# ronghanghu/speaker_follower

Measured on AMD Instinct MI355X. Metric: agent-steps/sec (follower rollout, batch 100), higher is better.
Workload: dtype f32; 1 GPU; follower rollout: batch 100 per GPU, 36 views x 2048-d features from a 10567-viewpoint HBM table, <=80-token instructions, 20 decode steps, argmax (student-forcing) feedback, every step executed for every row (no early exit), encoder included; global_batch=100, parallelism=dp1

## Files before the change

### include/sf_hip.h

```cpp
#ifndef SF_HIP_H_
#define SF_HIP_H_

#include <stddef.h>
#include <stdint.h>

#ifdef __cplusplus
extern "C" {
#endif

#define SF_ABI_VERSION 10

enum {
    SF_OK = 0,
    SF_ERR_ARG = 1,
    SF_ERR_UNSUPPORTED = 2,
    SF_ERR_LAUNCH = 3,
    SF_ERR_WORKSPACE = 4
};

typedef void* sf_stream;

typedef struct sf_dropout {
    float p;
    uint32_t seed;
// ... 397 lines not shown
                    float* logp, sf_stream stream);
int sf_scatter_rows(const float* src, int ld_src, const int32_t* idx, int n, int width, float* dst,
                    int ld_dst, sf_stream stream);

typedef struct sf_spk_beam {
    int32_t B, beam_size, k, T, Tp, eos;
    float* score;
    int64_t* words;
    int32_t* parent;
    int32_t* inst;
    int32_t* live_total;
    int32_t *hist_word, *hist_parent;
    float *hist_score, *hist_attn;
    int64_t ld_hist;
    int32_t* done_rec;
    float* done_score;
} sf_spk_beam;
int sf_speaker_beam_select(const sf_spk_beam* s, const int32_t* top_w, const float* top_lp, const float* alpha,
                           sf_stream stream);

#define SF_ROW_MOVES_MAX 4
typedef struct sf_row_move {
    const float* src;
    float* dst;
    const int32_t* idx;
    int32_t ld_src, ld_dst, width;
    int32_t scatter;
} sf_row_move;
int sf_move_rows(const sf_row_move* moves, int n_moves, int n, sf_stream stream);

int sf_fill_f32(float* p, size_t n, float v, sf_stream stream);
int sf_add_f32(float* dst, const float* src, size_t n, sf_stream stream);
#define SF_FILL_MAX_REGIONS 8
typedef struct sf_fill_region {
    void* ptr;
    uint64_t count;
    uint64_t value;
    int32_t width;
} sf_fill_region;
int sf_fill_regions(const sf_fill_region* regions, int n, sf_stream stream);
int sf_dropout_copy(const float* src, int lds, int B, int N, float* dst, int ldd,
                    const sf_dropout* drop, uint32_t drop_stream, int col0, sf_stream stream);
int sf_transpose(const float* src, int R, int Ccols, float* dst, sf_stream stream);
int sf_embedding_fwd(const float* table, int E, const int64_t* idx, int B, float* out,
                     sf_stream stream);

int sf_adam_step(float* p, const float* g, float* m, float* v, size_t n, double lr, double beta1,
                 double beta2, double eps, double weight_decay, int step, sf_stream stream);
int sf_adam_step_dev(float* p, const float* g, float* m, float* v, size_t n, double lr, double beta1, double beta2,
                     double eps, double weight_decay, int32_t* step_dev, float* coef, const uint32_t* skip_if_nonzero,
                     sf_stream stream);

void sf_debug_trace(unsigned long long* buf);
void sf_debug_force_write_through(int on);
void sf_debug_persist_timeout(long long ticks);
int sf_debug_cotenant(int blocks, int threads, int lds_bytes, long long ticks, float* sink, sf_stream stream);
void sf_gate_product_strict(int on);
int sf_gate_product_is_strict(void);
size_t sf_pack_bf16_bytes(int rows, int K);
int sf_pack_bf16(const float* w, int ld, int rows, int K, void* out, sf_stream stream);
int sf_lstm_weights_bf16(const float* w_ih, const float* w_hh, const void* packed_ih, const void* packed_hh);
void sf_gate_product_bf16_weights(int on);
int sf_gate_product_bf16_weights_is_on(void);
int sf_gate_product_bf16_supported(int M, int K1, int K2, int N);
int sf_feature_table_f16(const void* table, int on);
int sf_feature_table_is_f16(const void* table);
typedef struct sf_projected {
    const float *pv, *pa, *lv, *la;
    const float* loc_table;
    const float *key_v, *key_a;
    int32_t H, ld, V, IMG, LOC, reserved;
} sf_projected;
int sf_projected_ld(int H);
int sf_projected_build(const sf_decoder_fold* fold, const float* table, long long n_rows, const float* loc_table, int V, int IMG,
                       int LOC, int H, float* pv, float* pa, float* lv, float* la, void* ws, size_t ws_bytes,
                       sf_stream stream);
int sf_projected_register(const void* table, const sf_projected* p);
int sf_projected_registered(const void* table, sf_projected* out);
void sf_projected_use(int on);
int sf_projected_is_used(void);
long long sf_projected_steps(void);
int sf_projected_supported(int B, int H, int L, int A, int V, int IMG, int LOC);
void sf_debug_projected_chunk_rows(int rows);
void sf_debug_projected_partials_late(int on);
int sf_projected_text_groups_plan(int B, int L, int with_partials, int slots, int product_blocks, int* grid);
void sf_debug_projected_text_groups(int groups);
int sf_debug_projected_attention(const sf_pano* X, int B, int H, const float* pv, const float* lv, int ld, const float* h1,
                                 int ldh1, float* alpha, float* out, int ldo, int late, void* ws, size_t ws_bytes,
                                 sf_stream stream);
void sf_debug_gate_product_f32(int on);
void sf_debug_many_row_product(int on);
void sf_debug_grouped_weight_gradients(int on);
void sf_debug_slab_consumers(int on);
void sf_debug_precise_attention(int on);
void sf_debug_tn_split_min_rows(int rows);
size_t sf_workspace_fault_offset(size_t ws_bytes);
typedef struct sf_nav_table {
    const int32_t* a_num;
    const int32_t* next_row;
    const int32_t* cand_view;
    const float* cand_sincos;
    const int32_t* feat_row;
    int32_t A, V;
} sf_nav_table;
typedef struct sf_nav_io {
    sf_nav_table nav;
    const int32_t *row, *view;
    const int32_t* goal_hop;
    int32_t ld_hop;
    const int32_t* hop_base;
    int32_t *row_next, *vp_next, *view_next, *a_num_next;
    int32_t* cand_view_next;
    float* sincos_next;
    int64_t* target_next;
} sf_nav_io;
int sf_nav_step(const sf_nav_table* nav, int B, const int32_t* row, const int32_t* view,
                const int64_t* a_t, const uint8_t* ended, const int32_t* goal_hop, int ld_hop,
                const int32_t* hop_base, int32_t* row_next, int32_t* vp_next, int32_t* view_next,
                int32_t* a_num_next, int32_t* cand_view_next, float* sincos_next,
                int64_t* target_next, sf_stream stream);

typedef struct sf_fol_beam {
    int32_t B, beam_size, k, episode_len, T, reserved;
    sf_nav_table nav;
    float* score;
    int32_t *row, *view;
    int32_t* act;
    int32_t* parent;
    int32_t* inst;
    int32_t* live_total;
    int32_t *hist_parent, *hist_action, *hist_rank, *hist_sid, *hist_psid;
    float *hist_score, *hist_attn;
    int64_t ld_hist;
    int32_t* done_rec;
    float* done_score;
} sf_fol_beam;
int sf_follower_beam_select(const sf_fol_beam* s, const int32_t* top_a, const float* top_lp, const float* alpha,
                            sf_stream stream);

enum {
    SF_SEARCH_OVF_NODES = 1, SF_SEARCH_OVF_SLOTS = 2, SF_SEARCH_OVF_VISITS = 4, SF_SEARCH_OVF_POOL = 8,
    SF_SEARCH_OVF_KEY = 16
};
typedef struct sf_state_search {
    int32_t B, successor_size, completion_size, episode_len, key_fields, n_keys;
    int32_t node_cap, slot_cap, visit_cap, cap, pool_rows, reserved;
    sf_nav_table nav;
    const int32_t* base_row;
    int32_t* status;
    int32_t* inst;
    int32_t* frontier;
    int32_t *node_parent, *node_sid, *node_key, *node_action, *node_count, *node_pool, *node_start, *node_born;
    float* node_score;
    int32_t *open_slot, *open_key, *open_node;
    float* open_pick;
    int32_t *held_slot, *held_key, *held_node;
    float* held_pick;
    int32_t* comp_node;
    int32_t* comp_order;
    int32_t* visits;
} sf_state_search;
int sf_state_factored_select(const sf_state_search* s, const float* logp, int ld_logp, int32_t* dev_in,
                             sf_stream stream);

#define SF_EVAL_MAX_NODES 512
typedef struct sf_eval_graphs {
// ... 82 lines not shown
```

### speaker_follower_amd/csrc/sf_api.hip

```cpp
#include "sf_kernels.h"
#include "sf_gemm_small.h"
#include "sf_glue.h"

using namespace sf;

#include <atomic>
#include <climits>
#include <map>
#include <mutex>
#include <string>
#include <vector>

namespace sf {
thread_local hipError_t g_last_hip_error = hipSuccess;

namespace {
struct ProfRec { const char* name; hipEvent_t e0, e1; };
struct Prof {
    std::atomic<bool> active{false};
    std::vector<ProfRec> recs;
    std::vector<hipEvent_t> pool;
    size_t used = 0;
};
Prof g_prof;
std::mutex g_prof_mutex;
}
bool prof_active() { return g_prof.active.load(std::memory_order_acquire); }
void prof_events(const char* name, hipEvent_t* e0, hipEvent_t* e1) {
    std::lock_guard<std::mutex> lock(g_prof_mutex);
    Prof& p = g_prof;
    *e0 = *e1 = nullptr;
    if (!p.active.load(std::memory_order_relaxed)) return;
    while (p.pool.size() < p.used + 2) {
        hipEvent_t e = nullptr;
        if (hipEventCreate(&e) != hipSuccess) { e = nullptr; }
        p.pool.push_back(e);
    }
    if (!p.pool[p.used] || !p.pool[p.used + 1]) return;
    *e0 = p.pool[p.used++];
    *e1 = p.pool[p.used++];
    p.recs.push_back(ProfRec{name, *e0, *e1});
}
}

namespace {

constexpr size_t WORKSPACE_BYTES = 64u << 20;
constexpr size_t WGRAD_WORKSPACE_BYTES = 256u << 20;

struct Arena {
    float* base;
    size_t cap, off;
    unsigned* tk = nullptr;
    float* take(size_t n) {
        n = (n + 63) & ~(size_t)63;
        if (off + n > cap) return nullptr;
        float* p = base + off;
        off += n;
        return p;
    }
    float* rest() const { return base + off; }
    size_t rest_n() const { return cap - off; }
    unsigned* tickets() const { return tk; }
};
constexpr size_t SYNC_WORDS = 2048;
constexpr size_t PERSIST_TICKET = 1100;
constexpr size_t TEXT_TICKET = 1200;

inline Arena arena(void* ws, size_t bytes) {
    const size_t n = ws ? bytes / 4 : 0;
    const size_t usable = n > SYNC_WORDS ? n - SYNC_WORDS : 0;
    return Arena{(float*)ws, usable, 0, usable ? reinterpret_cast<unsigned*>((float*)ws + usable) : nullptr};
}
inline hipStream_t S(sf_stream s) { return (hipStream_t)s; }

constexpr int F16_TABLES = 16;
const void* g_f16_tables[F16_TABLES];
int g_f16_ntables = 0;
std::mutex g_f16_mutex;
int table_is_f16(const void* table) {
    if (!table) return 0;
    std::lock_guard<std::mutex> lock(g_f16_mutex);
    for (int i = 0; i < g_f16_ntables; ++i)
        if (g_f16_tables[i] == table) return 1;
    return 0;
}

constexpr int PROJ_TABLES = 16;
struct ProjEntry { const void* table; sf_projected p; };
ProjEntry g_proj[PROJ_TABLES];
int g_proj_n = 0;
std::mutex g_proj_mutex;
std::atomic<int> g_proj_use{1};
std::atomic<long long> g_proj_steps{0};
static int g_proj_partials_late = 0;
bool projected_lookup(const void* table, sf_projected* out) {
    if (!table || !g_proj_use.load(std::memory_order_relaxed)) return false;
    std::lock_guard<std::mutex> lock(g_proj_mutex);
    for (int i = 0; i < g_proj_n; ++i)
        if (g_proj[i].table == table) {
            *out = g_proj[i].p;
            return true;
        }
    return false;
}
inline int projected_ld(int H) { return (H + 1 + 3) & ~3; }

inline PanoSrc pano(const sf_pano* p) {
    return PanoSrc{p->dense, p->table, p->loc_table, p->vp, p->view, p->V, p->IMG, p->LOC,
                   p->dense ? 0 : table_is_f16(p->table)};
}
inline CandSrc cands(const sf_cands* c) {
    return CandSrc{c->dense, c->table, c->vp, c->cand_view, c->cand_sincos, c->a_num,
                   c->A, c->V, c->IMG, c->LOC, c->dense ? 0 : table_is_f16(c->table)};
}

inline FGlue make_glue(const CandSrc& src, int B, float* logit, const sf_follower_glue* g) {
    FGlue f{};
    f.src = src; f.B = B; f.logit = logit; f.is_valid = g->is_valid; f.target = g->target;
    f.feedback = g->feedback; f.ended = g->ended; f.a_t = g->a_t; f.target_used = g->target_used;
    f.score = g->score; f.u_next = g->u_next; f.ld_u = g->ld_u_next;
    f.u_drop = make_dropout(g->u_drop, g->u_drop_stream, 2);
    f.ce_term = g->ce_term; f.live = g->live; f.sample_seed = g->sample_seed;
    f.sample_stream = g->sample_stream; f.row0 = g->row0;
    f.sample_site = g->sample_site_dev ? g->sample_site_dev : site_zero();
    if (g->nav) {
        const sf_nav_io& n = *g->nav;
        f.nav = NavIO{n.nav, n.row, n.view, n.goal_hop, n.ld_hop, n.hop_base, n.row_next, n.vp_next, n.view_next,
                      n.a_num_next, n.cand_view_next, n.sincos_next, n.target_next, true};
    }
    return f;
}
inline bool glue_ok(const sf_cands* U, const sf_follower_glue* g) {
    return g->target && g->ended && g->a_t && g->target_used && g->score && g->ce_term && g->live &&
           g->feedback >= 0 && g->feedback <= 2 && (g->is_valid || U->a_num) &&
           (!g->u_next || g->ld_u_next % 4 == 0) &&
           (!g->nav || (g->nav->nav.A == U->A && g->nav->nav.a_num && g->nav->nav.next_row && g->nav->nav.cand_view &&
                        g->nav->nav.cand_sincos && g->nav->nav.feat_row && g->nav->row && g->nav->view &&
                        g->nav->row_next && g->nav->vp_next && g->nav->view_next && g->nav->a_num_next &&
                        g->nav->cand_view_next && g->nav->sincos_next &&
                        (!g->nav->target_next || (g->nav->goal_hop && g->nav->hop_base && g->nav->ld_hop > 0))));
}

#define TRY(expr)                     \
    do {                              \
        int _st = (expr);             \
        if (_st != SF_OK) return _st; \
    } while (0)
#define NEED(ptr) \
    if (!(ptr)) return SF_ERR_WORKSPACE

int colsum_pair(const float* Y, int ldy, int M, int N, float* a, float* b, Arena ar, hipStream_t st) {
    float* first = a ? a : b;
    if (!first) return SF_OK;
    return colsum(Y, ldy, M, N, first, 1, st, (a && b) ? b : nullptr, ar.rest(), ar.rest_n());
}

int linear_plain(const float* x, int ldx, const float* w, int ldw, const float* b, int M, int N,
                 int K, Epi epi, float* y, int ldy, Arena ar, hipStream_t st) {
    Seg sg{x, ldx, w, ldw, K};
    LinearOut o{};
    o.y = y;
    o.ldy = ldy;
    o.bias = b;
    o.epi = epi;
    return linear_nt(&sg, 1, M, N, o, ar.rest(), ar.rest_n(), st);
}

int data_grad(const float* dy, int lddy, const float* w, const float* w_t, int M, int N, int K,
              float* dx, int lddx, int accumulate, Arena ar, hipStream_t st) {
    if (w_t && N % 4 == 0) {
        Seg sg{dy, lddy, w_t, N, N};
        LinearOut o{};
        o.y = dx; o.ldy = lddx; o.epi = EPI_NONE; o.accumulate = accumulate;
        return linear_nt(&sg, 1, M, K, o, ar.rest(), ar.rest_n(), st);
    }
    return gemm_nn_ws(dy, lddy, w, K, M, K, N, dx, lddx, accumulate, ar.rest(), ar.rest_n(), st);
}

std::atomic<int> g_bf16w_on{0};
struct Bf16Pair { const float* w_ih; const float* w_hh; const void* p_ih; const void* p_hh; };
constexpr int BF16_PAIRS = 16;
Bf16Pair g_bf16_pairs[BF16_PAIRS];
int g_bf16_npairs = 0;
std::mutex g_bf16_mutex;

bool bf16_packed(const float* w_ih, const float* w_hh, const void* (&packed)[2]) {
    if (!g_bf16w_on.load(std::memory_order_relaxed) || sf::g_nt_force_f32) return false;
    std::lock_guard<std::mutex> lock(g_bf16_mutex);
    for (int i = 0; i < g_bf16_npairs; ++i)
        if (g_bf16_pairs[i].w_ih == w_ih && g_bf16_pairs[i].w_hh == w_hh) {
            packed[0] = g_bf16_pairs[i].p_ih;
            packed[1] = g_bf16_pairs[i].p_hh;
            return true;
        }
    return false;
}

int lstm_fwd_i(const sf_lstm_w* w, int B, int I, int H, const float* x, int ldx, const float* h0,
               const float* c0, float* h1, float* c1, float* gates, float* h1_drop, int ld_h1_drop,
               const Dropout& drop, Arena ar, hipStream_t st) {
    LstmPwFwd p{};
    p.xg = nullptr; p.b_ih = w->b_ih; p.b_hh = w->b_hh;
    p.c0 = c0; p.h0 = h0; p.B = B; p.H = H; p.gates = gates; p.h1 = h1; p.c1 = c1;
    p.h1_drop = h1_drop; p.ld_h1_drop = ld_h1_drop; p.drop = drop; p.lengths = nullptr;
    if (I + H <= 1024 && H % 16 == 0) {
        LstmStepArgs f{};
        f.h0 = h0; f.w_hh = w->w_hh; f.x = x; f.ldx = ldx; f.w_ih = w->w_ih; f.I = I; f.xg = nullptr;
        f.b_ih = w->b_ih; f.b_hh = w->b_hh; f.B = B; f.H = H; f.pw = p;
        return lstm_step_fused(f, st);
    }
    Seg segs[2] = {{x, ldx, w->w_ih, I, I}, {h0, H, w->w_hh, H, H}};
    LinearOut o{};
    float* slabs = nullptr;
    int ks = 1;
    const void* packed[2];
    const bool bf16w = bf16_packed(w->w_ih, w->w_hh, packed);
    TRY(linear_nt(segs, 2, B, 4 * H, o, ar.rest(), ar.rest_n(), st, &slabs, &ks, bf16w ? packed : nullptr));
    p.slabs = slabs; p.ks = ks;
    return lstm_pointwise_fwd(p, st);
}

static int g_slab_consumers = 1;

int lstm_bwd_i(const sf_lstm_w* w, const sf_lstm_g* g, int B, int I, int H, const float* x, int ldx,
               const float* h0, const float* c0, const float* c1, const float* gates,
               const float* dh1, const float* dh1_b, const float* dc1, float* dx, int lddx,
               float* dh0, float* dc0, Arena ar, hipStream_t st, float* dgates_out = nullptr,
               int dx_col0 = 0,
               const Dropout* dh1b_drop = nullptr,
               SmallPlan* dh0_plan = nullptr, bool* dh0_deferred = nullptr,
               const float** dx_slabs = nullptr, int* dx_ks = nullptr) {
    float* dgates = dgates_out ? dgates_out : ar.take((size_t)B * 4 * H);
    NEED(dgates);
    LstmPwBwd p{};
    p.gates = gates; p.c0 = c0; p.c1 = c1; p.dh1 = dh1; p.dh1_b = dh1_b; p.dc1 = dc1;
    p.B = B; p.H = H; p.dgates = dgates; p.dc0 = dc0; p.lengths = nullptr; p.dh0_pass = nullptr;
    if (dh1b_drop) p.dh1b_drop = *dh1b_drop;
    TRY(lstm_pointwise_bwd(p, st));
    if (dx && dx_col0 == 0) {
        TRY(data_grad(dgates, 4 * H, w->w_ih, w->w_ih_t, B, 4 * H, I, dx, lddx, 0, ar, st));
    } else if (dx) {
        const int I2 = I - dx_col0;
        if (dx_ks) *dx_ks = 0;
        if (w->w_ih_t) {
            Seg sg{dgates, 4 * H, w->w_ih_t + (size_t)dx_col0 * 4 * H, 4 * H, 4 * H};
            LinearOut o{};
            o.y = dx + dx_col0; o.ldy = lddx; o.epi = EPI_NONE;
            float* slabs = (dx_slabs && dx_ks && g_slab_consumers) ? ar.take((size_t)16 * B * I2) : nullptr;
            int ks = 0;
            float* raw = nullptr;
            if (slabs && linear_nt(&sg, 1, B, I2, o, slabs, (size_t)16 * B * I2, st, &raw, &ks) == SF_OK && raw == slabs && ks >= 1) {
                *dx_slabs = slabs;
                *dx_ks = ks;
            } else {
                TRY(linear_nt(&sg, 1, B, I2, o, ar.rest(), ar.rest_n(), st));
            }
        } else {
            TRY(gemm_nn_ws(dgates, 4 * H, w->w_ih + dx_col0, I, B, I2, 4 * H, dx + dx_col0, lddx, 0,
                           ar.rest(), ar.rest_n(), st));
        }
    }
    if (dh0_deferred) *dh0_deferred = false;
    if (dh0 && dh0_plan && dh0_deferred && w->w_hh_t) {
        Seg sg{dgates, 4 * H, w->w_hh_t, 4 * H, 4 * H};
        LinearOut o{};
        o.y = dh0; o.ldy = H; o.epi = EPI_NONE;
        *dh0_deferred = linear_small_plan(&sg, 1, B, H, o, dh0_plan);
    }
    if (dh0 && !(dh0_deferred && *dh0_deferred))
        TRY(data_grad(dgates, 4 * H, w->w_hh, w->w_hh_t, B, 4 * H, H, dh0, H, 0, ar, st));
    if (g) {
        if (g->w_ih) TRY(gemm_tn(dgates, 4 * H, x, ldx, B, 4 * H, I, g->w_ih, I, 1, st, ar.rest(), ar.rest_n()));
        if (g->w_hh) TRY(gemm_tn(dgates, 4 * H, h0, H, B, 4 * H, H, g->w_hh, H, 1, st, ar.rest(), ar.rest_n()));
        TRY(colsum_pair(dgates, 4 * H, B, 4 * H, g->b_ih, g->b_hh, ar, st));
    }
    return SF_OK;
}

int visual_fwd_i(const sf_visual_w* w, const PanoSrc& X, int B, int H, int D, const float* h,
                 float* out, int ldo, float* alpha, float* t_v, float* q, const Dropout& drop,
                 int col0, Arena ar, hipStream_t st, bool precise = false, const sf_visual_fold64* fold64 = nullptr) {
    const int F = X.IMG + X.LOC;
    if (precise && fold64 && fold64->m_v && fold64->c_v && visual_attn_f64_supported(X, B) && !(H & 3)) {
        double* q64 = reinterpret_cast<double*>(ar.take((size_t)B * F * 2));
        float* part = ar.take(visual_attn_split_floats(B, F));
        if (q64 && part && ar.tickets()) {
            TRY(linear_f64_w64(h, H, fold64->m_v, H, fold64->c_v, B, F, H, q64, F, q, F, st));
            return visual_attn(0, X, B, q, F, alpha, out, ldo, drop, col0, st, part, ar.tickets(), q64);
        }
    }
    if (precise && w->w_v_t && visual_attn_f64_supported(X, B) && !(H & 3) && !(D & 3)) {
        double* t64 = reinterpret_cast<double*>(ar.take((size_t)B * D * 2));
        double* q64 = reinterpret_cast<double*>(ar.take((size_t)B * F * 2));
        float* part = ar.take(visual_attn_split_floats(B, F));
        if (t64 && q64 && part && ar.tickets()) {
            TRY(linear_f64(h, nullptr, H, w->w_h, H, w->b_h, B, D, H, t64, D, t_v, D, st));
            TRY(linear_f64(nullptr, t64, D, w->w_v_t, D, nullptr, B, F, D, q64, F, q, F, st));
            return visual_attn(0, X, B, q, F, alpha, out, ldo, drop, col0, st, part, ar.tickets(), q64);
        }
// ... 228 lines not shown
        if (g_proj_n == PROJ_TABLES) return SF_ERR_UNSUPPORTED;
        at = g_proj_n++;
    }
    g_proj[at] = ProjEntry{table, *p};
    return SF_OK;
}
int sf_projected_registered(const void* table, sf_projected* out) {
    std::lock_guard<std::mutex> lock(g_proj_mutex);
    for (int i = 0; i < g_proj_n; ++i)
        if (table && g_proj[i].table == table) {
            if (out) *out = g_proj[i].p;
            return 1;
        }
    return 0;
}
void sf_projected_use(int on) { g_proj_use.store(on ? 1 : 0, std::memory_order_relaxed); }
int sf_projected_is_used(void) { return g_proj_use.load(std::memory_order_relaxed); }
long long sf_projected_steps(void) { return g_proj_steps.load(std::memory_order_relaxed); }
void sf_debug_projected_partials_late(int on) { g_proj_partials_late = on; }
void sf_debug_projected_text_groups(int groups) { sf::g_proj_text_groups = groups == 2 || groups == 4 ? groups : 0; }
int sf_projected_text_groups_plan(int B, int L, int with_partials, int slots, int product_blocks, int* grid) {
    if (B < 1 || L < 1 || slots < 0 || product_blocks < 0) return 0;
    return sf::proj_text_groups_plan(B, L, with_partials != 0, product_blocks, slots, 0, grid);
}
int sf_debug_projected_attention(const sf_pano* X, int B, int H, const float* pv, const float* lv, int ld, const float* h1,
                                 int ldh1, float* alpha, float* out, int ldo, int late, void* ws, size_t ws_bytes,
                                 sf_stream stream) {
    SF_ENTER();
    SF_CHECK_ARG(X && pv && lv && h1 && alpha && out && B > 0 && H > 0);
    const PanoSrc x = pano(X);
    Arena ar = arena(ws, ws_bytes);
    float* part = ar.take(visual_attn_split_floats(B, x.IMG + x.LOC));
    if (!part || !ar.tickets()) return SF_ERR_WORKSPACE;
    return proj_attention_alone(x, B, ProjTables{pv, nullptr, lv, nullptr, ld, H}, h1, ldh1, alpha, out, ldo, late, part,
                                ar.tickets(), S(stream));
}
constexpr long long PROJ_CHUNK_ROWS = 16384;
static long long g_proj_chunk_rows = PROJ_CHUNK_ROWS;
void sf_debug_projected_chunk_rows(int rows) { g_proj_chunk_rows = rows > 0 ? rows : PROJ_CHUNK_ROWS; }
int sf_projected_supported(int B, int H, int L, int A, int V, int IMG, int LOC) {
    if (H <= 0 || IMG <= 0 || LOC <= 0 || V <= 0) return 0;
    static const float dummy[4] = {0.f, 0.f, 0.f, 0.f};
    static const int idummy[1] = {0};
    CandSrc us{};
    us.table = dummy; us.a_num = idummy; us.A = A; us.V = V; us.IMG = IMG; us.LOC = LOC;
    PanoSrc xn{};
    xn.table = dummy; xn.V = V; xn.IMG = IMG; xn.LOC = LOC;
    const ProjTables pt{dummy, dummy, dummy, dummy, projected_ld(H), H};
    return proj_chain_supported(us, &xn, B, H, L, pt) ? 1 : 0;
}
int sf_projected_build(const sf_decoder_fold* fold, const float* table, long long n_rows, const float* loc_table, int V, int IMG,
                       int LOC, int H, float* pv, float* pa, float* lv, float* la, void* ws, size_t ws_bytes,
                       sf_stream stream) {
    SF_ENTER();
    SF_CHECK_ARG(fold && fold->m_v && fold->c_v && fold->m_a && fold->c_a && table && loc_table && pv && pa && lv && la &&
                 n_rows > 0 && V > 0 && IMG > 0 && IMG % 4 == 0 && LOC > 0 && LOC % 16 == 0 && H > 0 && H % 4 == 0);
    if (table_is_f16(table)) return SF_ERR_UNSUPPORTED;
    const int F = IMG + LOC, Fa = F + 4, ld = projected_ld(H), Ks = LOC + 4, g = LOC / 4;
    Arena ar = arena(ws, ws_bytes);
    hipStream_t st = S(stream);
    sf::proj_text_slots_warm();
    float* wt_v = ar.take((size_t)ld * F);
    float* wt_a = ar.take((size_t)ld * Fa);
    float* sel = ar.take((size_t)5 * Ks);
    NEED(wt_v && wt_a && sel);
    TRY(fill(wt_v + (size_t)H * F, (size_t)(ld - H) * F, 0.f, st));
    TRY(fill(wt_a + (size_t)H * Fa, (size_t)(ld - H) * Fa, 0.f, st));
    TRY(transpose(fold->m_v, F, H, wt_v, st));
    TRY(transpose(fold->m_a, Fa, H, wt_a, st));
    TRY(add2(fold->c_v, F, nullptr, 0, 1, F, wt_v + (size_t)H * F, F, st));
    TRY(add2(fold->c_a, Fa, nullptr, 0, 1, Fa, wt_a + (size_t)H * Fa, Fa, st));
    TRY(fill(sel, (size_t)5 * Ks, 0.f, st));
    for (int q = 0; q < 4; ++q) TRY(fill(sel + (size_t)q * Ks + (size_t)q * g, (size_t)g, 1.f, st));
    TRY(fill(sel + (size_t)4 * Ks + LOC, 1, 1.f, st));
    for (long long r0 = 0; r0 < n_rows; r0 += g_proj_chunk_rows) {
        const int m = (int)std::min<long long>(g_proj_chunk_rows, n_rows - r0);
        const float* x = table + (size_t)r0 * IMG;
        TRY(linear_plain(x, IMG, wt_v, F, nullptr, m, ld, IMG, EPI_NONE, pv + (size_t)r0 * ld, ld, ar, st));
        TRY(linear_plain(x, IMG, wt_a, Fa, nullptr, m, ld, IMG, EPI_NONE, pa + (size_t)r0 * ld, ld, ar, st));
    }
    TRY(linear_plain(loc_table, LOC, wt_v + IMG, F, nullptr, V * V, ld, LOC, EPI_NONE, lv, ld, ar, st));
    return linear_plain(sel, Ks, wt_a + IMG, Fa, nullptr, 5, ld, Ks, EPI_NONE, la, ld, ar, st);
}
void sf_gate_product_bf16_weights(int on) { g_bf16w_on.store(on ? 1 : 0, std::memory_order_relaxed); }
int sf_gate_product_bf16_weights_is_on(void) { return g_bf16w_on.load(std::memory_order_relaxed); }
int sf_gate_product_bf16_supported(int M, int K1, int K2, int N) {
    if (K2 < 0) return 0;
    const int K[2] = {K1, K2};
    return sf::bf16w_supported(M, N, K, K2 ? 2 : 1) ? 1 : 0;
}
void sf_debug_precise_attention(int on) { sf::g_precise_attention = on; }
void sf_debug_tn_split_min_rows(int rows) { sf::g_tn_split_min_rows = rows < 0 ? 4096 : rows; }
size_t sf_workspace_fault_offset(size_t ws_bytes) {
    const size_t n = ws_bytes / 4;
    if (n <= SYNC_WORDS) return 0;
    return (n - SYNC_WORDS + PERSIST_TICKET + persistent_fault_word()) * 4;
}
const char* sf_last_error_string(void) { return hipGetErrorString(g_last_hip_error); }
const char* sf_status_string(int s) {
    switch (s) {
        case SF_OK: return "ok";
        case SF_ERR_ARG: return "invalid argument";
        case SF_ERR_UNSUPPORTED: return "unsupported shape";
        case SF_ERR_LAUNCH: return "kernel launch failed";
        case SF_ERR_WORKSPACE: return "workspace too small";
        default: return "unknown status";
    }
}

int sf_linear_fwd(const float* x, int ldx, const float* w, const float* b, int M, int N, int K,
                  int act, float* y, int ldy, void* ws, size_t ws_bytes, sf_stream stream) {
    SF_ENTER();
    SF_CHECK_ARG(x && w && y && M > 0 && N > 0 && K > 0 && (act == 0 || act == 1));
    return linear_plain(x, ldx, w, K, b, M, N, K, act ? EPI_TANH : EPI_NONE, y, ldy,
                        arena(ws, ws_bytes), S(stream));
}

int sf_linear_slabs_fwd(const float* x, int ldx, const float* w, int K1, const float* h, int ldh,
                        const float* u, int K2, int M, int N, int* ksplit, void* ws, size_t ws_bytes,
                        sf_stream stream) {
    SF_ENTER();
    SF_CHECK_ARG(x && w && ksplit && ws && M > 0 && N > 0 && K1 > 0 && (!h || (u && K2 > 0)));
    Arena ar = arena(ws, ws_bytes);
    Seg segs[2] = {{x, ldx, w, K1, K1}, {h, ldh, u, K2, K2}};
    LinearOut o{};
    float* slabs = nullptr;
    const void* packed[2];
    const bool bf16w = bf16_packed(w, h ? u : nullptr, packed);
    return linear_nt(segs, h ? 2 : 1, M, N, o, ar.rest(), ar.rest_n(), S(stream), &slabs, ksplit, bf16w ? packed : nullptr);
}

int sf_linear_bwd(const float* x, int ldx, const float* w, const float* y, int ldy, const float* dy,
                  int lddy, int M, int N, int K, int act, float* dx, int lddx, int accumulate_dx,
                  float* dw, float* db, void* ws, size_t ws_bytes, sf_stream stream) {
    SF_ENTER();
    SF_CHECK_ARG(x && w && dy && M > 0 && N > 0 && K > 0 && (N % 4 == 0) && (K % 4 == 0));
    Arena ar = arena(ws, ws_bytes);
    hipStream_t st = S(stream);
    const float* dpre = dy;
    int ldp = lddy;
    if (act == 1) {
        SF_CHECK_ARG(y);
        float* t = ar.take((size_t)M * N);
        NEED(t);
        TRY(tanh_bwd(y, ldy, dy, lddy, M, N, t, N, st));
        dpre = t;
        ldp = N;
    }
    if (dx) TRY(gemm_nn_ws(dpre, ldp, w, K, M, K, N, dx, lddx, accumulate_dx, ar.rest(), ar.rest_n(), st));
    if (dw) TRY(gemm_tn(dpre, ldp, x, ldx, M, N, K, dw, K, 1, st, ar.rest(), ar.rest_n()));
    if (db) TRY(colsum(dpre, ldp, M, N, db, 1, st, nullptr, ar.rest(), ar.rest_n()));
    return SF_OK;
}

int sf_lstm_cell_fwd(const sf_lstm_w* w, int B, int I, int H, const float* x, int ldx,
                     const float* h0, const float* c0, float* h1, float* c1, float* gates,
                     float* h1_drop, int ld_h1_drop, const sf_dropout* drop, uint32_t drop_stream,
                     void* ws, size_t ws_bytes, sf_stream stream) {
    SF_ENTER();
    SF_CHECK_ARG(w && x && h0 && c0 && h1 && c1 && B > 0 && I > 0 && H > 0 && H % 4 == 0);
    return lstm_fwd_i(w, B, I, H, x, ldx, h0, c0, h1, c1, gates, h1_drop, ld_h1_drop,
                      make_dropout(drop, drop_stream), arena(ws, ws_bytes), S(stream));
}

int sf_lstm_cell_bwd(const sf_lstm_w* w, const sf_lstm_g* g, int B, int I, int H, const float* x,
                     int ldx, const float* h0, const float* c0, const float* c1, const float* gates,
// ... 68 lines not shown
    SF_ENTER();
    SF_CHECK_ARG(w && ctx && alpha && cat2 && t_text && h_tilde && dh_tilde && dh && B > 0);
    return softdot_bwd_i(w, g, B, L, H, ctx, alpha, cat2, t_text, h_tilde, dh_tilde, dh, lddh, dctx,
                         arena(ws, ws_bytes), S(stream));
}

int sf_text_attention_fwd(const float* ctx, const uint8_t* mask, int B, int L, int H, const float* t, int ldt,
                          float* alpha, float* wc, int ldwc, sf_stream stream) {
    SF_ENTER();
    SF_CHECK_ARG(ctx && t && alpha && wc && B > 0 && L > 0 && H > 0);
    return text_attn_fwd(ctx, mask, B, L, H, t, ldt, alpha, wc, ldwc, S(stream));
}

int sf_text_attention_bwd(const float* ctx, int B, int L, int H, const float* dwc, int lddwc, const float* t, int ldt,
                          const float* alpha, float* dt, int lddt, float* dctx, sf_stream stream) {
    SF_ENTER();
    SF_CHECK_ARG(ctx && dwc && t && alpha && dt && B > 0 && L > 0 && H > 0);
    return text_attn_bwd(ctx, B, L, H, dwc, lddwc, t, ldt, alpha, dt, lddt, dctx, S(stream));
}

int sf_eltwise_prod_scoring_fwd(const sf_scoring_w* w, const sf_cands* U, int B, int H, int D,
                                const float* h, float* logit, float* t_a, float* wt, float* r,
                                void* ws, size_t ws_bytes, sf_stream stream) {
    SF_ENTER();
    SF_CHECK_ARG(w && U && h && logit && t_a && wt && r && B > 0);
    return scoring_fwd_i(w, cands(U), B, H, D, h, logit, t_a, wt, r, arena(ws, ws_bytes), S(stream));
}

int sf_eltwise_prod_scoring_bwd(const sf_scoring_w* w, const sf_scoring_g* g, const sf_cands* U,
                                int B, int H, int D, const float* h, const float* t_a,
                                const float* wt, const float* dlogit, float* dh, void* ws,
                                size_t ws_bytes, sf_stream stream) {
    SF_ENTER();
    SF_CHECK_ARG(w && U && h && t_a && wt && dlogit && B > 0);
    return scoring_bwd_i(w, g, cands(U), B, H, D, h, t_a, wt, dlogit, dh, arena(ws, ws_bytes),
                         S(stream));
}

static int decoder_head_a(const sf_decoder_w* w, const sf_pano* X, int B, int H, int D,
                          const float* h0, const sf_decoder_tape* tp, const sf_dropout* drop,
                          uint32_t step_id, Arena ar, sf_stream stream) {
    SF_CHECK_ARG(w && X && h0 && tp && B > 0);
    const PanoSrc xs = pano(X);
    const int F = xs.IMG + xs.LOC;
    return visual_fwd_i(&w->visual, xs, B, H, D, h0, tp->xin + F, 2 * F, tp->alpha_v, tp->t_v, tp->q,
                        make_dropout(drop, 2 * step_id, 2), F, ar, S(stream));
}

int sf_attn_decoder_head_fwd(const sf_decoder_w* w, const sf_pano* X, int B, int H, int D,
                             const float* h0, const sf_decoder_tape* tp, const sf_dropout* drop,
                             uint32_t step_id, void* ws, size_t ws_bytes, sf_stream stream) {
    SF_ENTER();
    return decoder_head_a(w, X, B, H, D, h0, tp, drop, step_id, arena(ws, ws_bytes), stream);
}

static int plan_linear(const float* x, int ldx, const float* wgt, int ldw, const float* b, int M,
                       int N, int K, Epi epi, float* y, int ldy, SmallPlan* p) {
    Seg sg{x, ldx, wgt, ldw, K};
    LinearOut o{};
    o.y = y; o.ldy = ldy; o.bias = b; o.epi = epi;
    return linear_small_plan(&sg, 1, M, N, o, p) ? SF_OK : SF_ERR_UNSUPPORTED;
}

struct TextFold {
    const float* ctx_q;
    const float* ctx_o;
};

struct TailStep {
    const sf_decoder_w* w;
    CandSrc us;
    int B, H, D, L, F;
    const sf_decoder_tape *tp, *tn;
    const sf_follower_glue* glue;
    Dropout d_h, dn_in;
    PanoSrc xn;
    bool has_xn;
    bool paired, query_only, last_step;
    const float* ctx;
    const uint8_t* ctx_mask;
    const int32_t* ctx_row;
    Arena ar;
    hipStream_t st;
};

static inline int issued(int rc) { return rc == SF_ERR_UNSUPPORTED ? SF_ERR_LAUNCH : rc; }

static SmallPlan empty_plan(SmallPlan p) {
    p.gx = p.gy = 0;
    return p;
}

static int vis_next_beside(const TailStep& s, float* part, unsigned* counter, const SmallPlan& b, int phase = 0) {
    return pair_vis_small(s.xn, s.B, s.tn->q, s.F, s.tn->alpha_v, s.tn->xin + s.F, 2 * s.F, s.dn_in, s.F, part, counter, b,
                          s.st, phase);
}
static int vis_next_alone(const TailStep& s, float* part, const Arena& ar) {
    return visual_attn(0, s.xn, s.B, s.tn->q, s.F, s.tn->alpha_v, s.tn->xin + s.F, 2 * s.F, s.dn_in, s.F, s.st, part,
                       part ? ar.tickets() : nullptr);
}

static int score_tail(const TailStep& s, const Arena& ar, bool t_a_done = false) {
    const sf_decoder_tape* tp = s.tp;
    return scoring_fwd_i(&s.w->action, s.us, s.B, s.H, s.D, tp->h_tilde, tp->logit, tp->t_a, tp->wt, tp->r, ar, s.st, s.glue,
                         t_a_done);
}

struct FoldScratch {
    float *tpart, *ybuf, *zbuf, *part;
    unsigned* tcount;
    int ldp;
    bool ok;
};
static FoldScratch fold_scratch(const TailStep& s, Arena& af) {
    FoldScratch f{};
    f.tpart = af.take(text_fold_part_floats(s.B, s.H));
    f.ldp = s.H + 16;
    f.ybuf = af.take((size_t)s.B * f.ldp);
    f.zbuf = af.take((size_t)s.B * f.ldp);
    f.tcount = af.tickets() ? af.tickets() + TEXT_TICKET : nullptr;
    f.part = (s.paired && s.B <= 1024) ? af.take(visual_attn_split_floats(s.B, s.F)) : nullptr;
    f.ok = f.tpart && f.ybuf && f.zbuf && (f.part || !s.paired) && f.tcount && s.B <= VIS_SPLIT_MAX_B;
    return f;
}

static int fold_score(const TailStep& s, float* merge_part) {
    const sf_scoring_w& a = s.w->action;
    const sf_decoder_tape* tp = s.tp;
    if (merge_part)
        return pair_score_merge(s.us, s.B, s.D, tp->r, tp->wt, a.b_a, a.b_out, make_glue(s.us, s.B, tp->logit, s.glue), s.xn,
                                s.tn->alpha_v, s.tn->xin + s.F, 2 * s.F, s.dn_in, s.F, merge_part, s.st);
    if (s.glue)
        return score_glue_fwd(s.us, s.B, s.D, tp->r, tp->wt, a.b_a, a.b_out, make_glue(s.us, s.B, tp->logit, s.glue), s.st);
    return score_fwd(s.us, s.B, s.D, tp->r, tp->wt, a.b_a, a.b_out, tp->logit, s.st);
}

static bool projected_for(const sf_decoder_w* w, const CandSrc& us, const PanoSrc* xn, int B, int H, int L, ProjTables* pt) {
    sf_projected reg;
    if (us.dense || us.half || !projected_lookup(us.table, &reg)) return false;
    if (reg.key_v != w->visual.w_h || reg.key_a != w->action.w_h || reg.V != us.V || reg.IMG != us.IMG || reg.LOC != us.LOC ||
        (xn && xn->loc_table != reg.loc_table))
        return false;
    *pt = ProjTables{reg.pv, reg.pa, reg.lv, reg.la, reg.ld, reg.H};
    return proj_chain_supported(us, xn, B, H, L, *pt);
}

static int tail_proj(const TailStep& s, const TextFold& tf) {
    const sf_decoder_tape *tp = s.tp, *tn = s.tn;
    const int B = s.B, H = s.H, F = s.F;
    ProjTables pt;
    if (!s.glue || s.query_only || !(s.paired || s.last_step) ||
        !projected_for(s.w, s.us, s.paired ? &s.xn : nullptr, B, H, s.L, &pt))
        return SF_ERR_UNSUPPORTED;
    Arena af = s.ar;
    const FoldScratch f = fold_scratch(s, af);
    SmallPlan py;
    const bool ok = f.ok &&
        plan_linear(tp->cat2 + H, 2 * H, s.w->text.w_out + H, 2 * H, nullptr, B, H, H, EPI_NONE, f.ybuf, f.ldp, &py) == SF_OK &&
        pair_proj_textfold_accepts(py.inst()) && (!s.paired || af.tickets());
    if (!ok) return SF_ERR_UNSUPPORTED;
    const bool late = s.paired && (g_proj_partials_late || !proj_partials_supported(s.xn.IMG, s.xn.LOC));
    TRY(pair_proj_textfold(tf.ctx_q, tf.ctx_o, s.ctx_mask, B, s.L, H, tp->cat2 + H, 2 * H, f.tpart, f.tcount, f.zbuf, f.ldp,
                           tp->alpha, py, s.us, s.paired && !late ? &s.xn : nullptr, pt, tp->h1, H, f.part, s.st));
    g_proj_steps.fetch_add(1, std::memory_order_relaxed);
    return issued(pair_proj_score(s.us, B, H, s.L, pt, f.zbuf, f.ldp, f.ybuf, f.ldp, make_glue(s.us, B, tp->logit, s.glue),
                                  s.paired ? &s.xn : nullptr, late ? 0 : 2, tp->h1, H, s.paired ? tn->alpha_v : nullptr,
                                  s.paired ? tn->xin + F : nullptr, 2 * F, s.dn_in, F, f.part, af.tickets(), s.st));
}

static int tail_fold4(const TailStep& s, const TextFold& tf) {
    const sf_visual_w* vw = &s.w->visual;
    const sf_scoring_w* aw = &s.w->action;
    const sf_decoder_tape *tp = s.tp, *tn = s.tn;
    const int B = s.B, H = s.H, D = s.D, F = s.F;
    Arena af = s.ar;
    const FoldScratch f = fold_scratch(s, af);
    SmallPlan py, pv, pta, pq, pr;
    bool ok = f.ok &&
        plan_linear(tp->cat2 + H, 2 * H, s.w->text.w_out + H, 2 * H, nullptr, B, H, H, EPI_NONE, f.ybuf, f.ldp, &py) == SF_OK &&
        plan_linear(tp->wt, D, aw->w_a_t, D, nullptr, B, F, D, EPI_NONE, tp->r, F, &pr) == SF_OK;
    if (ok && !s.last_step) {
        ok = plan_linear(tp->h1, H, vw->w_h, H, vw->b_h, B, D, H, EPI_NONE, tn->t_v, D, &pv) == SF_OK &&
             plan_linear(tn->t_v, D, vw->w_v_t, D, nullptr, B, F, D, EPI_NONE, tn->q, F, &pq) == SF_OK;
    } else if (ok) {
        pv = empty_plan(py);
        pq = empty_plan(pr);
    }
    if (ok) {
        Seg sg{f.ybuf, f.ldp, aw->w_h, H, H};
        LinearOut o{};
        o.y = tp->wt; o.ldy = D; o.bias = aw->b_h; o.mul = aw->w_out; o.y_pre = tp->t_a;
        o.ldy_pre = D; o.epi = EPI_MUL;
        ok = linear_small_plan(&sg, 1, B, D, o, &pta) && pair_apro_small_accepts(pta.inst(), pq.inst()) &&
             pair_vis_small_accepts(pr.inst(), 1);
        pta.args.apro_part = f.zbuf;
        pta.args.apro_stride = f.ldp;
    }
    if (!ok) return SF_ERR_UNSUPPORTED;
    TRY(pair_textfold_small_small(tf.ctx_q, tf.ctx_o, s.ctx_mask, B, s.L, H, tp->cat2 + H, 2 * H, f.tpart, f.tcount, f.zbuf,
                                  f.ldp, tp->alpha, py, pv, s.st));
    TRY(issued(pair_apro_small(pta, pq, s.st)));
    const bool merge_late = s.paired && s.glue;
    if (merge_late) TRY(issued(vis_next_beside(s, f.part, nullptr, pr, 1)));
    else if (s.paired) TRY(issued(vis_next_beside(s, f.part, af.tickets(), pr, 0)));
    else TRY(issued(launch_small_plan(pr, s.st)));
    return issued(fold_score(s, merge_late ? f.part : nullptr));
}

static int text_and_query(const TailStep& s) {
    const sf_softdot_w* tw = &s.w->text;
    const sf_visual_w* vw = &s.w->visual;
    const sf_decoder_tape *tp = s.tp, *tn = s.tn;
    const int B = s.B, H = s.H, D = s.D, L = s.L, F = s.F;
    SmallPlan pa, pb;
    const bool ok1 =
        plan_linear(tp->cat2 + H, 2 * H, tw->w_in, H, nullptr, B, H, H, EPI_NONE, tp->t_text, H, &pa) == SF_OK &&
        plan_linear(tp->h1, H, vw->w_h, H, vw->b_h, B, D, H, EPI_NONE, tn->t_v, D, &pb) == SF_OK;
    if (!ok1 || pair_small_small(pa, pb, s.st) != SF_OK) {
        TRY(linear_plain(tp->cat2 + H, 2 * H, tw->w_in, H, nullptr, B, H, H, EPI_NONE, tp->t_text, H, s.ar, s.st));
        TRY(linear_plain(tp->h1, H, vw->w_h, H, vw->b_h, B, D, H, EPI_NONE, tn->t_v, D, s.ar, s.st));
    }
    const bool ok2 = plan_linear(tn->t_v, D, vw->w_v_t, D, nullptr, B, F, D, EPI_NONE, tn->q, F, &pa) == SF_OK;
    if (!ok2 || pair_small_text(pa, s.ctx, s.ctx_mask, B, L, H, tp->t_text, H, tp->alpha, tp->cat2,
                                2 * H, s.ctx_row, s.st) != SF_OK) {
        TRY(text_attn_fwd(s.ctx, s.ctx_mask, B, L, H, tp->t_text, H, tp->alpha, tp->cat2, 2 * H, s.st, s.ctx_row));
        TRY(linear_plain(tn->t_v, D, vw->w_v_t, D, nullptr, B, F, D, EPI_NONE, tn->q, F, s.ar, s.st));
    }
    return SF_OK;
}

static int tail_paired(const TailStep& s) {
    const sf_softdot_w* tw = &s.w->text;
    const sf_scoring_w* aw = &s.w->action;
    const sf_decoder_tape* tp = s.tp;
    const int B = s.B, H = s.H, D = s.D, F = s.F;
    Arena ar = s.ar;
    float* part = B <= 1024 ? ar.take(visual_attn_split_floats(B, F)) : nullptr;
    SmallPlan ph, pc;
    const bool ok3 = part && plan_linear(tp->cat2, 2 * H, tw->w_out, 2 * H, nullptr, B, H, 2 * H,
                                         EPI_TANH, tp->h_tilde, H, &ph) == SF_OK;
    bool ok4 = false;
    if (ok3) {
        Seg sg{tp->h_tilde, H, aw->w_h, H, H};
        LinearOut o{};
        o.y = tp->wt; o.ldy = D; o.bias = aw->b_h; o.mul = aw->w_out; o.y_pre = tp->t_a;
        o.ldy_pre = D; o.epi = EPI_MUL;
        ok4 = linear_small_plan(&sg, 1, B, D, o, &pc) && pair_vis_small_accepts(pc.inst(), 2);
    }
    TRY(text_and_query(s));
    if (ok4 && vis_next_beside(s, part, nullptr, ph, 1) == SF_OK) {
        TRY(vis_next_beside(s, part, nullptr, pc, 2));
        return score_tail(s, ar, true);
    }
    if (!ok3 || vis_next_beside(s, part, ar.tickets(), ph) != SF_OK) {
        TRY(linear_plain(tp->cat2, 2 * H, tw->w_out, 2 * H, nullptr, B, H, 2 * H, EPI_TANH, tp->h_tilde, H, ar, s.st));
        TRY(vis_next_alone(s, part, ar));
    }
    return score_tail(s, ar);
}

static int tail_query_only(const TailStep& s) {
    const sf_decoder_tape* tp = s.tp;
    TRY(text_and_query(s));
    TRY(linear_plain(tp->cat2, 2 * s.H, s.w->text.w_out, 2 * s.H, nullptr, s.B, s.H, 2 * s.H, EPI_TANH, tp->h_tilde, s.H,
                     s.ar, s.st));
    return score_tail(s, s.ar);
}

static int tail_plain(const TailStep& s) {
    const sf_decoder_tape *tp = s.tp, *tn = s.tn;
    TRY(softdot_fwd_i(&s.w->text, s.B, s.L, s.H, nullptr, 0, s.ctx, s.ctx_mask, tp->h_tilde, tp->alpha, tp->cat2,
                      tp->t_text, s.ar, s.st, s.ctx_row));
    if (s.has_xn)
        TRY(visual_fwd_i(&s.w->visual, s.xn, s.B, s.H, s.D, tp->h1, tn->xin + s.F, 2 * s.F, tn->alpha_v, tn->t_v, tn->q,
                         s.dn_in, s.F, s.ar, s.st));
    return score_tail(s, s.ar);
}

static int tail_dispatch(const TailStep& s, const TextFold* tf) {
    const bool foldable = (s.paired || s.query_only || s.last_step) && tf && !s.ctx_row && !s.d_h.on() && s.w->text.w_out;
    int rc = SF_ERR_UNSUPPORTED;
    if (foldable) rc = tail_proj(s, *tf);
    if (rc == SF_ERR_UNSUPPORTED && foldable && s.w->action.w_a_t) rc = tail_fold4(s, *tf);
    if (rc != SF_ERR_UNSUPPORTED) return rc;
    if (s.paired) return tail_paired(s);
    if (s.query_only) return tail_query_only(s);
    return tail_plain(s);
}

static int decoder_tail_i(const sf_decoder_w* w, const sf_cands* U, int B, int H, int D, int L,
                          const float* u_prev, const float* h0, const float* c0, const float* ctx,
                          const uint8_t* ctx_mask, const int32_t* ctx_row, const sf_decoder_tape* tp,
                          const sf_follower_glue* glue, const sf_dropout* drop, uint32_t step_id,
                          const sf_pano* X_next, const sf_decoder_tape* tn, void* ws, size_t ws_bytes,
                          sf_stream stream, const TextFold* tf = nullptr) {
    SF_CHECK_ARG(w && U && h0 && c0 && ctx && tp && B > 0 && L > 0 && (!glue || glue_ok(U, glue)) &&
                 (!X_next || tn));
    TailStep s{};
    s.w = w; s.us = cands(U); s.B = B; s.H = H; s.D = D; s.L = L; s.F = s.us.IMG + s.us.LOC;
    s.tp = tp; s.tn = tn; s.glue = glue;
    s.ctx = ctx; s.ctx_mask = ctx_mask; s.ctx_row = ctx_row;
    s.ar = arena(ws, ws_bytes);
    s.st = S(stream);
    s.d_h = make_dropout(drop, 2 * step_id + 1, 2);
    s.dn_in = make_dropout(drop, 2 * (step_id + 1), 2);
    s.has_xn = X_next != nullptr;
    if (X_next) s.xn = pano(X_next);
    s.paired = X_next && w->visual.w_v_t;
    s.query_only = !X_next && tn && w->visual.w_v_t;
    s.last_step = !X_next && !tn;
    const Dropout d_in = make_dropout(drop, 2 * step_id, 2);
    if (u_prev) TRY(dropout_copy(u_prev, s.F, B, s.F, tp->xin, 2 * s.F, d_in, 0, s.st));
    TRY(lstm_fwd_i(&w->lstm, B, 2 * s.F, H, tp->xin, 2 * s.F, h0, c0, tp->h1, tp->c1, tp->gates,
                   tp->cat2 + H, 2 * H, s.d_h, s.ar, s.st));
    return tail_dispatch(s, tf);
}

static int decoder_tail_split_i(const sf_decoder_w* w, const sf_cands* U, int B, int H, int D, int L,
                                const float* h0, const float* c0, const float* ctx, const uint8_t* ctx_mask,
                                const sf_decoder_tape* tp, const sf_follower_glue* glue, const sf_dropout* drop,
                                uint32_t step_id, unsigned* flag_h1, unsigned flag_value, void* ws,
                                size_t ws_bytes, unsigned* tickets, hipStream_t st) {
    SF_CHECK_ARG(w && U && h0 && c0 && ctx && tp && glue && glue_ok(U, glue));
    const size_t n = ws_bytes / 4;
    Arena ar{(float*)ws, n, 0, tickets};
    const CandSrc us = cands(U);
    const int F = us.IMG + us.LOC;
    const Dropout d_h = make_dropout(drop, 2 * step_id + 1, 2);
    TRY(lstm_fwd_i(&w->lstm, B, 2 * F, H, tp->xin, 2 * F, h0, c0, tp->h1, tp->c1, tp->gates, tp->cat2 + H, 2 * H,
                   d_h, ar, st));
    if (flag_h1) TRY(flag_set(flag_h1, flag_value, st));
    TRY(softdot_fwd_i(&w->text, B, L, H, nullptr, 0, ctx, ctx_mask, tp->h_tilde, tp->alpha, tp->cat2, tp->t_text,
                      ar, st, nullptr));
    return scoring_fwd_i(&w->action, us, B, H, D, tp->h_tilde, tp->logit, tp->t_a, tp->wt, tp->r, ar, st, glue);
}

int sf_attn_decoder_attend_fwd(const sf_pano* X, int B, const sf_decoder_tape* tp, const sf_dropout* drop,
                               uint32_t step_id, void* ws, size_t ws_bytes, sf_stream stream) {
    SF_ENTER();
    SF_CHECK_ARG(X && tp && tp->q && tp->xin && tp->alpha_v && B > 0);
    Arena ar = arena(ws, ws_bytes);
    const PanoSrc xs = pano(X);
    const int F = xs.IMG + xs.LOC;
    float* part = B <= 1024 ? ar.take(visual_attn_split_floats(B, F)) : nullptr;
    return visual_attn(0, xs, B, tp->q, F, tp->alpha_v, tp->xin + F, 2 * F, make_dropout(drop, 2 * step_id, 2), F,
                       S(stream), part, part ? ar.tickets() : nullptr);
}

int sf_attn_decoder_tail_fwd(const sf_decoder_w* w, const sf_cands* U, int B, int H, int D, int L,
                             const float* u_prev, const float* h0, const float* c0,
                             const float* ctx, const uint8_t* ctx_mask, const int32_t* ctx_row,
                             const sf_decoder_tape* tp, const sf_follower_glue* glue,
                             const sf_dropout* drop, uint32_t step_id, const sf_pano* X_next,
                             const sf_decoder_tape* tn, void* ws, size_t ws_bytes,
                             sf_stream stream) {
    SF_ENTER();
    return decoder_tail_i(w, U, B, H, D, L, u_prev, h0, c0, ctx, ctx_mask, ctx_row, tp, glue, drop,
                          step_id, X_next, tn, ws, ws_bytes, stream);
}

int sf_attn_decoder_fwd(const sf_decoder_w* w, const sf_pano* X, const sf_cands* U, int B, int H,
                        int D, int L, const float* u_prev, const float* h0, const float* c0,
                        const float* ctx, const uint8_t* ctx_mask, const int32_t* ctx_row,
                        const sf_decoder_tape* tp, const sf_follower_glue* glue,
                        const sf_dropout* drop, uint32_t step_id,
                        void* ws, size_t ws_bytes, sf_stream stream) {
    SF_ENTER();
    SF_CHECK_ARG(w && X && U && h0 && c0 && ctx && tp && B > 0 && L > 0 && (!glue || glue_ok(U, glue)));
    TRY(decoder_head_a(w, X, B, H, D, h0, tp, drop, step_id, arena(ws, ws_bytes), stream));
    return decoder_tail_i(w, U, B, H, D, L, u_prev, h0, c0, ctx, ctx_mask, ctx_row, tp, glue, drop, step_id, nullptr,
                          nullptr, ws, ws_bytes, stream);
}

int sf_decoder_fold_build(const sf_decoder_w* w, int H, int D, int F, float* m_v, float* c_v,
                          float* m_a, float* c_a, void* ws, size_t ws_bytes, sf_stream stream) {
    SF_ENTER();
    SF_CHECK_ARG(w && m_v && c_v && m_a && c_a && w->visual.w_v_t && w->visual.w_h_t &&
                 w->action.w_a_t && w->action.w_h_t && F % 4 == 0 && D % 4 == 0 && H % 4 == 0);
    Arena ar = arena(ws, ws_bytes);
    hipStream_t st = S(stream);
    float* wa_s = ar.take((size_t)F * D);
    float* wo_ba = ar.take(D);
    float* wo_bh = ar.take(D);
    NEED(wa_s && wo_ba && wo_bh);
    TRY(linear_plain(w->visual.w_v_t, D, w->visual.w_h_t, D, nullptr, F, H, D, EPI_NONE, m_v, H, ar, st));
    TRY(linear_plain(w->visual.b_h, D, w->visual.w_v_t, D, nullptr, 1, F, D, EPI_NONE, c_v, F, ar, st));
    TRY(scale_cols(w->action.w_a_t, D, w->action.w_out, F, D, wa_s, D, st));
    TRY(scale_cols(w->action.b_a, D, w->action.w_out, 1, D, wo_ba, D, st));
    TRY(scale_cols(w->action.b_h, D, w->action.w_out, 1, D, wo_bh, D, st));
    TRY(fill(m_a + (size_t)F * H, (size_t)4 * H, 0.f, st));
    TRY(fill(c_a + F, 4, 0.f, st));
    TRY(linear_plain(wa_s, D, w->action.w_h_t, D, nullptr, F, H, D, EPI_NONE, m_a, H, ar, st));
    TRY(linear_plain(wo_ba, D, w->action.w_h_t, D, nullptr, 1, H, D, EPI_NONE, m_a + (size_t)F * H, H, ar, st));
    TRY(linear_plain(wo_bh, D, w->action.w_a_t, D, nullptr, 1, F, D, EPI_NONE, c_a, F + 4, ar, st));
    return linear_plain(wo_bh, D, w->action.b_a, D, w->action.b_out, 1, 1, D, EPI_NONE, c_a + F, 4, ar, st);
}

// ... 197 lines not shown
        side = side_st;
        ev_join = ev_back;
        return SF_OK;
    }
    int join() {
        hipStream_t from = side;
        side = nullptr;
        return order_behind(main, from, ev_join);
    }
    ~SideFork() { if (side) (void)join(); }
};
}
}

int sf_follower_episode_fwd(const sf_decoder_w* w, const sf_follower_episode* e, void* ws,
                            size_t ws_bytes, sf_stream stream) {
    SF_ENTER();
    SF_CHECK_ARG(w && e && e->S > 0 && e->B > 0 && e->h_init && e->c_init && e->ctx && e->tape.xin &&
                 e->tape.h1 && e->tape.c1 && e->glue.target && e->glue.ended);
    const sf_dropout* drop = e->drop.p > 0.f ? &e->drop : nullptr;
    StepView cur = step_view(e, 0);
    TextFold tfold{e->ctx_q, e->ctx_o};
    const TextFold* tf = nullptr;
    if (e->ctx_q && e->ctx_o && !drop && e->S > 1 && w->text.w_in_t && w->text.w_out && w->action.w_a_t) {
        const int M = e->B * e->L, H = e->H;
        const Arena ar = arena(ws, ws_bytes);
        TRY(linear_plain(e->ctx, H, w->text.w_in_t, H, nullptr, M, H, H, EPI_NONE, e->ctx_q, H, ar, S(stream)));
        TRY(linear_plain(e->ctx, H, w->text.w_out, 2 * H, nullptr, M, H, H, EPI_NONE, e->ctx_o, H, ar, S(stream)));
        tf = &tfold;
    }
    {
        Arena ha = arena(ws, ws_bytes);
        const PanoSrc x0 = pano(&cur.X);
        ProjTables pt;
        float* part = nullptr;
        bool head_done = false;
        if (tf && !e->glue.nav && e->B <= VIS_SPLIT_MAX_B && projected_for(w, cands(&cur.U), &x0, e->B, e->H, e->L, &pt) &&
            (part = ha.take(visual_attn_split_floats(e->B, x0.IMG + x0.LOC))) && ha.tickets()) {
            const int F = x0.IMG + x0.LOC;
            const int rc = visual_attn_proj(cands(&cur.U), x0, e->B, e->H, e->L, pt, e->h_init, e->H, cur.tp.alpha_v,
                                            cur.tp.xin + F, 2 * F, make_dropout(drop, 2 * e->step0, 2), F, part, ha.tickets(),
                                            S(stream));
            if (rc == SF_OK) head_done = true;
            else if (rc != SF_ERR_UNSUPPORTED) return rc;
        }
        if (!head_done)
            TRY(decoder_head_a(w, &cur.X, e->B, e->H, e->D, e->h_init, &cur.tp, drop, e->step0, ha, stream));
    }
    const sf_nav_io* nav0 = e->glue.nav;
    if (nav0) SF_CHECK_ARG(w->visual.w_v_t);
    if (!nav0 && e->side_stream && e->side_stream != stream && e->S > 1 && !tf) {
        hipStream_t ms = S(stream), ss = S(e->side_stream);
        std::vector<hipEvent_t>& ev = event_pool(2);
        if (ev.size() < 2) return SF_ERR_LAUNCH;
        const Arena whole = arena(ws, ws_bytes);
        if (!whole.tk) return SF_ERR_WORKSPACE;
        const size_t side_n = std::min<size_t>(whole.cap / 4, (size_t)4 << 20);
        unsigned* flag_h1 = whole.tk + PERSIST_TICKET + 48;
        unsigned* flag_ft = whole.tk + PERSIST_TICKET + 49;
        void* side_ws = (float*)ws + (whole.cap - side_n);
        const size_t main_bytes = (whole.cap - side_n) * sizeof(float);
        TRY(flag_set(flag_h1, 0u, ms));
        TRY(flag_set(flag_ft, 0u, ms));
        SideFork fk{ms};
        TRY(fk.fork(ss, ev[0], ev[1]));
        for (int t = 0; t < e->S; ++t) {
            const bool more = t + 1 < e->S;
            StepView nxt = more ? step_view(e, t + 1) : cur;
            const StepState in = state_in(e, t);
            if (t > 0) TRY(flag_wait(flag_ft, (unsigned)t, ms));
            TRY(decoder_tail_split_i(w, &cur.U, e->B, e->H, e->D, e->L, in.h, in.c, e->ctx, e->ctx_mask, &cur.tp,
                                     &cur.glue, drop, e->step0 + t, more ? flag_h1 : nullptr, (unsigned)(t + 1), ws,
                                     main_bytes, whole.tk, ms));
            if (more) {
                TRY(flag_wait(flag_h1, (unsigned)(t + 1), ss));
                Arena sar{(float*)side_ws, side_n, 0, whole.tk};
                TRY(decoder_head_a(w, &nxt.X, e->B, e->H, e->D, cur.tp.h1, &nxt.tp, drop, e->step0 + t + 1, sar, e->side_stream));
                TRY(flag_set(flag_ft, (unsigned)(t + 1), ss));
            }
            cur = nxt;
        }
        return fk.join();
    }
    for (int t = 0; t < e->S; ++t) {
        const bool more = t + 1 < e->S;
        StepView nxt = more ? step_view(e, t + 1) : cur;
        const sf_nav_io nv = nav0 ? nav_view(nav0, e, t) : sf_nav_io{};
        if (nav0) cur.glue.nav = &nv;
        const StepState in = state_in(e, t);
        TRY(decoder_tail_i(w, &cur.U, e->B, e->H, e->D, e->L, nullptr, in.h, in.c, e->ctx, e->ctx_mask,
                           nullptr, &cur.tp, &cur.glue, drop, e->step0 + t, more && !nav0 ? &nxt.X : nullptr,
                           more ? &nxt.tp : nullptr, ws, ws_bytes, stream, tf));
        if (nav0 && more)
            TRY(sf_attn_decoder_attend_fwd(&nxt.X, e->B, &nxt.tp, drop, e->step0 + t + 1, ws, ws_bytes, stream));
        cur = nxt;
    }
    return SF_OK;
}

int sf_follower_episode_bwd(const sf_decoder_w* w, const sf_follower_episode* e,
                            const sf_decoder_gtape* gtape, const float* gscale, float* dlogit,
                            float* dh_a, float* dc_a, float* dh_b, float* dc_b, float* dctx,
                            int* result_in_b, void* ws, size_t ws_bytes, sf_stream stream) {
    SF_ENTER();
    SF_CHECK_ARG(w && e && gtape && gscale && dlogit && dh_a && dc_a && dh_b && dc_b && result_in_b &&
                 e->S > 0 && e->B > 0);
    const sf_dropout* drop = e->drop.p > 0.f ? &e->drop : nullptr;
    sf_decoder_gtape gt_all = *gtape;
    if (!(gt_all.dcat2 && gt_all.ds && dctx && ctx_grad_supported(e->S, e->L, e->H)))
        gt_all.dcat2 = gt_all.ds = nullptr;
    gtape = &gt_all;
    const float *dh1 = nullptr, *dc1 = nullptr;
    float *dho = dh_a, *dco = dc_a, *dhn = dh_b, *dcn = dc_b;
    hipStream_t main_st = S(stream), side_st = S(e->side_stream);
    const bool two = side_st && side_st != main_st && gtape->dh1d && gtape->dcat2 && gtape->ds &&
                     e->B <= VIS_SPLIT_MAX_B;
    if (two) {
        SF_CHECK_ARG(e->ctx && dctx);
        std::vector<hipEvent_t>& ev = event_pool(e->S + 1);
        if (ev.size() < (size_t)e->S + 1) return SF_ERR_LAUNCH;
        const Arena whole = arena(ws, ws_bytes);
        const size_t usable = whole.cap;
        const size_t head_n = std::min<size_t>(usable / 4, (size_t)4 << 20);
        Arena tail_ar{(float*)ws, usable - head_n, 0, whole.tk};
        Arena head_ar{(float*)ws + (usable - head_n), head_n, 0, whole.tk};
        TRY(order_behind(side_st, main_st, ev[e->S]));
        for (int t = e->S - 1; t >= 0; --t) {
            StepView v = step_view(e, t);
            const sf_decoder_gtape g = gtape_view(gtape, e, t);
            const CeSrc ce{v.tp.logit, v.glue.target_used, gscale + t, -1, (int)e->A};
            TRY(decoder_bwd_head_i(w, nullptr, &v.U, e->B, e->H, e->D, e->L, e->ctx, &v.tp, &g, dlogit,
                                   g.dh1d, dctx, head_ar, side_st, &ce));
            if (hipEventRecord(ev[t], side_st) != hipSuccess) return SF_ERR_LAUNCH;
        }
        for (int t = e->S - 1; t >= 0; --t) {
            StepView v = step_view(e, t);
            const sf_decoder_gtape g = gtape_view(gtape, e, t);
            const StepState in = state_in(e, t);
            if (hipStreamWaitEvent(main_st, ev[t], 0) != hipSuccess) return SF_ERR_LAUNCH;
            TRY(decoder_bwd_tail_i(w, nullptr, &v.X, e->B, e->H, e->D, in.h, in.c, &v.tp, &g, dh1, g.dh1d, dc1,
                                   dho, dco, drop, e->step0 + t, tail_ar, main_st));
            dh1 = dho;
            dc1 = dco;
            std::swap(dho, dhn);
            std::swap(dco, dcn);
        }
    } else {
        for (int t = e->S - 1; t >= 0; --t) {
            StepView v = step_view(e, t);
            const sf_decoder_gtape g = gtape_view(gtape, e, t);
            const StepState in = state_in(e, t);
            const CeSrc ce{v.tp.logit, v.glue.target_used, gscale + t, -1, (int)e->A};
            TRY(decoder_bwd_i(w, nullptr, &v.X, &v.U, e->B, e->H, e->D, e->L, in.h, in.c, e->ctx, &v.tp, &g,
                              dlogit, dh1, dc1, dho, dco, dctx, drop, e->step0 + t, ws, ws_bytes, stream,
                              &ce));
            dh1 = dho;
            dc1 = dco;
            std::swap(dho, dhn);
            std::swap(dco, dcn);
        }
    }
    *result_in_b = (dh1 == dh_b) ? 1 : 0;
    if (gtape->dcat2 && gtape->ds && dctx)
        TRY(ctx_grad_accum(e->tape.alpha, gtape->ds, gtape->dcat2, 2 * e->H, e->tape.t_text, e->S, e->B,
                           e->L, e->H, dctx, S(stream)));
    return SF_OK;
}

int sf_attn_decoder_wgrad(const sf_decoder_w* w, const sf_decoder_g* g, int M, int H, int D, int F,
                          const float* h0_all, const sf_decoder_tape* tp, const sf_decoder_gtape* gt,
                          void* ws, size_t ws_bytes, sf_stream stream) {
    SF_ENTER();
    SF_CHECK_ARG(w && g && h0_all && tp && gt && M > 0);
    hipStream_t st = S(stream);
    Arena ar = arena(ws, ws_bytes);
// ... 980 lines not shown
```

### speaker_follower_amd/csrc/sf_attention.hip

```cpp
#include <atomic>
#include "sf_kernels.h"
#include "sf_rows.h"
#include "sf_glue.h"
#include "sf_gemm_small.h"

namespace sf {

namespace {


struct VisArgs {
    PanoSrc src;
    const float* vec;
    int ldvec;
    float* alpha;
    float* out;
    int ldo;
    Dropout drop;
    int drop_col0;
    const double* vec64;
    int vec_slabs;
    long vec_slab_stride;
    const float* pv;
    const float* lv;
// ... 823 lines not shown
        dlv = a.logit[(size_t)b * A + min(lane, A - 1)];
    }
    const CandRow row = cand_row<H16>(a.src, b, wave);
    float4 p[SC_CPL];
#pragma unroll
    for (int i = 0; i < SC_CPL; ++i) p[i] = f4zero();
    if (wave < A && !row.zero && w != 0.f) {
#pragma unroll
        for (int i = 0; i < SC_CPL; ++i) {
            const int c = lane + 64 * i;
            f4fma(p[i], w, cand_load<H16>(row, c, c < n4, n4));
        }
    }
    if (wave == 0) {
        const float tot = wave_sum(lane < A ? dlv : 0.f);
        if (lane == 0) a.dc[b] = tot;
    }
    float* orow = a.dr + (size_t)b * (n4 << 2);
    block_row_sum<SC_CPL, SC_NW, SC_SLOTS>(p, slots, n4, [&](int c, float4 t) {
        reinterpret_cast<float4*>(orow)[c] = t;
    });
}

template <int MTA, int CPWA, int MTB, int CPWB>
__global__ __launch_bounds__(SMALL_WAVES * 64) void pair_small_small_kernel(SmallArgs a, int gxa,
                                                                           int na, SmallArgs b,
                                                                           int gxb) {
    const int bid = blockIdx.x;
    if (bid < na)
        small_gemm_body<MTA, CPWA>(a, bid % gxa, bid / gxa);
    else
        small_gemm_body<MTB, CPWB>(b, (bid - na) % gxb, (bid - na) / gxb);
}

template <int MT, int CPW, int RPW>
__global__ __launch_bounds__(TXT_NW * 64) void pair_small_text_kernel(SmallArgs a, int gxa, int na,
                                                                      TxtArgs t) {
    const int bid = blockIdx.x;
    if (bid < na) {
        if (threadIdx.x >= SMALL_WAVES * 64) return;
        small_gemm_body<MT, CPW>(a, bid % gxa, bid / gxa);
    } else {
        text_attn_body<RPW, 0>(t, bid - na);
    }
}

template <int MT, int CPW, int PHASE, bool APRO = false, bool H16 = false>
__global__ __launch_bounds__(SMALL_WAVES * 64) void pair_vis_small_kernel(VisArgs v, VisSplit sp,
                                                                         int nv, SmallArgs b,
                                                                         int gxb) {
    const int bid = blockIdx.x;
    if (bid < nv) {
        if (threadIdx.x >= VSP_NW * 64) return;
        if (PHASE == 2)
            visual_split_body<2>(v, sp, 0, bid);
        else
            visual_split_body<PHASE, false, H16>(v, sp, bid % VSP_G, bid / VSP_G);
    } else {
        small_gemm_body<MT, CPW, false, APRO>(b, (bid - nv) % gxb, (bid - nv) / gxb);
    }
}


template <bool H16>
__global__ __launch_bounds__(SC_NW * 64) void pair_score_merge_kernel(ScoreArgs a, FGlue g, int nb, VisArgs v, VisSplit sp) {
    const int bid = blockIdx.x;
    if (bid < nb) {
        score_glue_body<H16>(a, g, bid);
    } else {
        if (threadIdx.x >= VSP_NW * 64) return;
        visual_split_body<2>(v, sp, 0, bid - nb);
    }
}


struct ProjScoreArgs {
    CandSrc src;
    const float* pa;
    const float* la;
    int ldp, H;
    const float* z;
    const float* y;
    int ldz, ldy;
};

__device__ __forceinline__ void proj_score_glue_body(const ProjScoreArgs& a, const FGlue& g, int b) {
    constexpr int NW = SMALL_WAVES, SLOTS = 2;
    __shared__ float s_logit[64];
    __shared__ int s_at;
    const int tid = threadIdx.x, lane = tid & 63, wave = tid >> 6;
    const int A = a.src.A, V = a.src.V, H = a.H, n4h = H >> 2;
    const size_t ldp = (size_t)a.ldp;
    const FGlueIn gin = follower_glue_load(g, b);
    const int vp = a.src.vp[b], an = a.src.a_num[b];
    const int cvl = a.src.cand_view[(size_t)b * A + min(lane, A - 1)];
    const float4 scl = reinterpret_cast<const float4*>(a.src.cand_sincos)[(size_t)b * A + min(lane, A - 1)];
    float4 zv[PRJ_CPL], yv[PRJ_CPL], lav[5][PRJ_CPL], pav[SLOTS][PRJ_CPL];
    float lac[5], pac[SLOTS];
#pragma unroll
    for (int i = 0; i < PRJ_CPL; ++i) {
        const int cc = min(lane + 64 * i, n4h - 1);
        zv[i] = reinterpret_cast<const float4*>(a.z + (size_t)b * a.ldz)[cc];
        yv[i] = reinterpret_cast<const float4*>(a.y + (size_t)b * a.ldy)[cc];
#pragma unroll
        for (int q = 0; q < 5; ++q) lav[q][i] = reinterpret_cast<const float4*>(a.la + q * ldp)[cc];
    }
#pragma unroll
    for (int q = 0; q < 5; ++q) lac[q] = a.la[q * ldp + H];
#pragma unroll
    for (int k = 0; k < SLOTS; ++k) {
        const int view = __shfl(cvl, min(wave + NW * k, A - 1), WAVE);
        const float* pr = a.pa + ((size_t)max(vp, 0) * V + min(max(view, 0), V - 1)) * ldp;
#pragma unroll
        for (int i = 0; i < PRJ_CPL; ++i) pav[k][i] = reinterpret_cast<const float4*>(pr)[min(lane + 64 * i, n4h - 1)];
        pac[k] = pr[H];
    }
    float4 ht[PRJ_CPL];
#pragma unroll
    for (int i = 0; i < PRJ_CPL; ++i) ht[i] = lane + 64 * i < n4h ? apro_form(yv[i], zv[i]) : f4zero();
#pragma unroll
    for (int k = 0; k < SLOTS; ++k) {
        const int ac = wave + NW * k, acc = min(ac, A - 1);
        const float s0 = __shfl(scl.x, acc, WAVE), s1 = __shfl(scl.y, acc, WAVE), s2 = __shfl(scl.z, acc, WAVE),
                    s3 = __shfl(scl.w, acc, WAVE);
        const float hm = (ac < A && ac != 0 && ac < an && vp >= 0) ? 1.f : 0.f;
        float d = 0.f;
#pragma unroll
        for (int i = 0; i < PRJ_CPL; ++i) {
            float4 w = pav[k][i];
            f4fma(w, s0, lav[0][i]);
            f4fma(w, s1, lav[1][i]);
            f4fma(w, s2, lav[2][i]);
            f4fma(w, s3, lav[3][i]);
            float4 t = lav[4][i];
            f4fma(t, hm, w);
            d += dot4(t, ht[i]);
        }
        d = wave_sum(d);
        const float cst = lac[4] + hm * (pac[k] + s0 * lac[0] + s1 * lac[1] + s2 * lac[2] + s3 * lac[3]);
        if (lane == 0 && ac < A) s_logit[ac] = d + cst;
    }
    __syncthreads();
    if (wave == 0) {
        const int at = follower_glue_row(g, b, lane < A ? s_logit[lane] : 0.f, gin);
        if (lane == 0) s_at = at;
        if (g.nav.on && lane < A) nav_advance_slot(g.nav, b, lane, at, gin.was_ended || at == 0);
    }
    __syncthreads();
    if (g.u_next) {
        const int at = min(max(s_at, 0), A - 1);
        const int n4 = (a.src.IMG + a.src.LOC) >> 2;
        CandRow row;
        row.zero = at == 0 || at >= an || vp < 0;
        row.I4 = a.src.IMG >> 2;
        row.g4 = max(a.src.LOC >> 4, 1);
        const int view = __shfl(cvl, at, WAVE);
        row.img = reinterpret_cast<const float4*>(a.src.table) + ((size_t)max(vp, 0) * V + min(max(view, 0), V - 1)) * row.I4;
        row.img16 = nullptr;
        row.s0 = __shfl(scl.x, at, WAVE); row.s1 = __shfl(scl.y, at, WAVE);
        row.s2 = __shfl(scl.z, at, WAVE); row.s3 = __shfl(scl.w, at, WAVE);
        for (int c = tid; c < n4; c += NW * 64) store_u_next(g, b, c, cand_load<false>(row, c, !row.zero, n4));
    }
}

template <int VPHASE>
__global__ __launch_bounds__(SMALL_WAVES * 64) void pair_proj_score_kernel(ProjScoreArgs a, FGlue g, int nb, VisArgs v, VisSplit sp,
                                                                         int nv) {
    const int bid = blockIdx.x;
    if (VPHASE == 0) {
        if (bid >= nv) return proj_score_glue_body(a, g, bid - nv);
        if (threadIdx.x >= VSP_NW * 64) return;
        visual_split_body<0, false, false, true>(v, sp, bid % VSP_G, bid / VSP_G);
    } else {
        if (bid < nb) return proj_score_glue_body(a, g, bid);
        proj_merge_body<PPB_G, PPB_RPG>(v, sp, bid - nb);
    }
}


struct TxtFoldArgs {
    const float* ctx_q;
    const float* ctx_o;
    const uint8_t* mask;
    int L, H;
    const float* vec;
    int ldvec;
    float* part;
    unsigned* counter;
    float* z;
    int ldz;
    float* alpha;
};

template <int RPW, int G>
__device__ __forceinline__ void text_fold_body(const TxtFoldArgs& a, int g, int b) {
    constexpr int NW = SMALL_WAVES, SL = 4, LG = NW * RPW;
    static_assert(LG <= 62, "a group's weights live in 62 record slots");
    static_assert(G >= 1 && G <= TXF_G && TXF_G % G == 0, "a launch adds TXF_G tickets per sample; the scratch holds TXF_G");
    typedef unsigned v4u __attribute__((ext_vector_type(4)));
    __shared__ float4 slots[SL][TXT_CPL * 64];
    __shared__ float s_score[LG];
    __shared__ int s_last;
    const int tid = threadIdx.x, lane = tid & 63, wave = tid >> 6;
    const int L = a.L, H = a.H, n4 = H >> 2;
    const int pstride = H + 64;
    const float4* cq = reinterpret_cast<const float4*>(a.ctx_q) + (size_t)b * L * n4;
    const float4* co = reinterpret_cast<const float4*>(a.ctx_o) + (size_t)b * L * n4;
    const bool use_mask = a.mask != nullptr;
    const uint8_t* mrow = use_mask ? a.mask + (size_t)b * L : reinterpret_cast<const uint8_t*>(cq);
    const int lt = g * LG + tid;
    const bool padded = tid >= LG || lt >= L || (use_mask && mrow[min(lt, L - 1)] != 0);
    const bool empty = __syncthreads_and(padded) != 0;
    float m = -INFINITY, e = 0.f, lsum = 0.f;
    float4 p[TXT_CPL];
#pragma unroll
    for (int i = 0; i < TXT_CPL; ++i) p[i] = f4zero();
    if (!empty) {
    float4 xq[RPW][TXT_CPL], xo[RPW][TXT_CPL];
    uint8_t mk[RPW];
#pragma unroll
    for (int r = 0; r < RPW; ++r) {
        const int l = g * LG + wave * RPW + r;
        const int lc = min(l, L - 1);
#pragma unroll
        for (int i = 0; i < TXT_CPL; ++i) {
            const int c = lane + 64 * i;
            const float4 tq = cq[(size_t)lc * n4 + min(c, n4 - 1)];
            const float4 to = co[(size_t)lc * n4 + min(c, n4 - 1)];
            const bool ok = l < L && c < n4;
            xq[r][i] = ok ? tq : f4zero();
            xo[r][i] = ok ? to : f4zero();
        }
        mk[r] = mrow[lc];
    }
    float4 v[TXT_CPL];
#pragma unroll
    for (int i = 0; i < TXT_CPL; ++i) {
        const int c = lane + 64 * i;
        const float4 t = reinterpret_cast<const float4*>(a.vec + (size_t)b * a.ldvec)[min(c, n4 - 1)];
        v[i] = c < n4 ? t : f4zero();
    }
#pragma unroll
    for (int r = 0; r < RPW; ++r) {
        float d = 0.f;
// ... 340 lines not shown
    if (half_misuse(src)) return SF_ERR_ARG;
    VisArgs va{src, vec, ldvec, alpha, out, ldo, drop, drop_col0, nullptr, vec_slabs, vec_slab_stride};
    const int nb = b.gx * b.gy;
    SF_LAUNCH_INST_H16(src.half, pair_visbwd_small_kernel, (1, 16), dim3(B + nb), dim3(VIS_NW * 64), 0, st, va, B, b.args, b.gx);
    return launch_status();
}

bool proj_chain_supported(const CandSrc& us, const PanoSrc* xn, int B, int H, int L, const ProjTables& pt) {
    if (!pt.pv || !pt.pa || !pt.lv || !pt.la || !us.table || !us.a_num) return false;
    if (xn && (xn->table != us.table || xn->V != us.V)) return false;
    const RowShape x = xn ? shape(*xn) : RowShape{};
    return proj_chain_supported(shape(us), xn ? &x : nullptr, B, H, L, pt.H, pt.ld);
}

static VisArgs proj_vis_args(const PanoSrc& xn, const ProjTables& pt, const float* h1, int ldh1, float* alpha, float* out,
                             int ldo, const Dropout& drop, int drop_col0) {
    VisArgs va{xn, h1, ldh1, alpha, out, ldo, drop, drop_col0};
    va.pv = pt.pv; va.lv = pt.lv; va.ldp = pt.ld; va.pH = pt.H;
    return va;
}

int visual_attn_proj(const CandSrc& us, const PanoSrc& x, int B, int H, int L, const ProjTables& pt, const float* h, int ldh,
                     float* alpha, float* out, int ldo, const Dropout& drop, int drop_col0, float* split_part,
                     unsigned* counter, hipStream_t st) {
    if (!proj_chain_supported(us, &x, B, H, L, pt) || !aligned4(ldh, ldo) || !split_part || !counter) return SF_ERR_UNSUPPORTED;
    const VisArgs va = proj_vis_args(x, pt, h, ldh, alpha, out, ldo, drop, drop_col0);
    SF_LAUNCH(visual_attn_split_proj_kernel, dim3(VSP_G, B), dim3(VSP_NW * 64), 0, st, va, VisSplit{split_part, counter, nullptr});
    return launch_status();
}

int g_proj_text_groups = 0;
static_assert(TXF_G == 4, "pair_proj_textfold names its instantiations <R, true, 2> and <R, true, 4>");
static int proj_text_slots(int rung) {
    constexpr int kMaxDev = 64;
    static std::atomic<int> cache[kMaxDev][4];
    int dev = 0;
    if (hipGetDevice(&dev) != hipSuccess || dev < 0 || dev >= kMaxDev) {
        (void)hipGetLastError();
        return 0;
    }
    if (cache[dev][0].load(std::memory_order_acquire) == 0) {
        int cus = 0, per[4] = {0, 0, 0, 0};
        bool ok = hipDeviceGetAttribute(&cus, hipDeviceAttributeMultiprocessorCount, dev) == hipSuccess;
#define SF_OCC(i, R)                                                                                               \
    ok = ok && hipOccupancyMaxActiveBlocksPerMultiprocessor(&per[i], pair_proj_textfold_kernel<R, true, TXF_G>,   \
                                                            SMALL_WAVES * 64, 0) == hipSuccess
        SF_OCC(0, 1); SF_OCC(1, 2); SF_OCC(2, 3); SF_OCC(3, 5);
#undef SF_OCC
        if (!ok) (void)hipGetLastError();
        for (int r = 3; r >= 0; --r)
            cache[dev][r].store((ok && cus > 0 && per[r] > 0 ? cus * per[r] : 0) + 1, std::memory_order_release);
    }
    return cache[dev][rung].load(std::memory_order_acquire) - 1;
}
void proj_text_slots_warm() { (void)proj_text_slots(0); }

int pair_proj_textfold(const float* ctx_q, const float* ctx_o, const uint8_t* mask, int B, int L, int H, const float* vec,
                       int ldvec, float* part, unsigned* counter, float* z, int ldz, float* alpha, const SmallPlan& y,
                       const CandSrc& us, const PanoSrc* xn, const ProjTables& pt, const float* h1, int ldh1, float* split_part,
                       hipStream_t st) {
    if (!pair_proj_textfold_accepts(y.inst()) || !proj_chain_supported(us, xn, B, H, L, pt)) return SF_ERR_UNSUPPORTED;
    if (!aligned4(ldvec, ldh1, ldz) || !counter || !z || ldz < H || (xn && !split_part)) return SF_ERR_UNSUPPORTED;
    if (xn && !proj_partials_supported(xn->IMG, xn->LOC)) return SF_ERR_UNSUPPORTED;
    const TxtFoldArgs ta{ctx_q, ctx_o, mask, L, H, vec, ldvec, part, counter, z, ldz, alpha};
    const VisArgs va = xn ? proj_vis_args(*xn, pt, h1, ldh1, nullptr, nullptr, 0, Dropout{}, 0) : VisArgs{};
    const VisSplit sp{split_part, nullptr, g_trace};
    const int nv = xn ? PPB_G * B : 0, na = y.gx * y.gy;
    const int force = g_proj_text_groups;
    const int slots = xn && L <= TXF_G2_MAX_L && force == 0 ? proj_text_slots(text_rung(L, TXF_G)) : 0;
    int blocks = 0;
    const int G = proj_text_groups_plan(B, L, xn != nullptr, na, slots, force, &blocks);
    const int nt = G * B;
    const dim3 grid(blocks), block(SMALL_WAVES * 64);
    return launched(with_index(fold_rpw(L, G), [&](auto r) {
        constexpr int R = decltype(r)::value;
        if (nv && G == 2) SF_LAUNCH_INST(pair_proj_textfold_kernel, (R, true, 2), grid, block, 0, st, va, sp, nv, ta, nt, y.args, y.gx);
        else if (nv) SF_LAUNCH_INST(pair_proj_textfold_kernel, (R, true, 4), grid, block, 0, st, va, sp, nv, ta, nt, y.args, y.gx);
        else SF_LAUNCH_INST(pair_proj_textfold_kernel, (R, false), grid, block, 0, st, va, sp, nv, ta, nt, y.args, y.gx);
    }, ints<1, 2, 3, 5>{}));
}

int pair_proj_score(const CandSrc& us, int B, int H, int L, const ProjTables& pt, const float* z, int ldz, const float* y, int ldy,
                    const FGlue& g, const PanoSrc* xn, int vphase, const float* h1, int ldh1, float* alpha, float* out, int ldo,
                    const Dropout& drop, int drop_col0, float* split_part, unsigned* counter, hipStream_t st) {
    if (!proj_chain_supported(us, xn, B, H, L, pt) || !aligned4(ldz, ldy, ldh1)) return SF_ERR_UNSUPPORTED;
    if (xn && (!split_part || !aligned4(ldo) || (vphase != 0 && vphase != 2) || (vphase == 0 && !counter))) return SF_ERR_UNSUPPORTED;
    const ProjScoreArgs a{us, pt.pa, pt.la, pt.ld, H, z, y, ldz, ldy};
    const VisArgs va = xn ? proj_vis_args(*xn, pt, h1, ldh1, alpha, out, ldo, drop, drop_col0) : VisArgs{};
    const VisSplit sp{split_part, counter, g_trace};
    const dim3 block(SMALL_WAVES * 64);
    if (xn && vphase == 0)
        SF_LAUNCH((pair_proj_score_kernel<0>), dim3(VSP_G * B + B), block, 0, st, a, g, B, va, sp, VSP_G * B);
    else
        SF_LAUNCH((pair_proj_score_kernel<2>), dim3(xn ? 2 * B : B), block, 0, st, a, g, B, va, sp, 0);
    return launch_status();
}

int proj_attention_alone(const PanoSrc& x, int B, const ProjTables& pt, const float* h1, int ldh1, float* alpha, float* out,
                         int ldo, int late, float* split_part, unsigned* counter, hipStream_t st) {
    if (x.dense || x.half || !x.table || !x.loc_table || !x.vp || !x.view || !pt.pv || !pt.lv || !h1 || !alpha || !out ||
        !split_part)
        return SF_ERR_ARG;
    if (B < 1 || !split_rows_fit(shape(x), B) || !proj_tables_fit(pt.H, pt.ld) || !aligned4(ldh1, ldo) || ldh1 < pt.H ||
        ldo < x.IMG + x.LOC || (late ? !counter : !proj_partials_supported(x.IMG, x.LOC)))
        return SF_ERR_UNSUPPORTED;
    const VisArgs va = proj_vis_args(x, pt, h1, ldh1, alpha, out, ldo, Dropout{}, 0);
    const VisSplit sp{split_part, late ? counter : nullptr, nullptr};
    const dim3 block(SMALL_WAVES * 64);
    if (late) {
        SF_LAUNCH((pair_proj_score_kernel<0>), dim3(VSP_G * B), block, 0, st, ProjScoreArgs{}, FGlue{}, 0, va, sp, VSP_G * B);
    } else {
        SF_LAUNCH((pair_proj_textfold_kernel<1, true>), dim3(PPB_G * B), block, 0, st, va, sp, PPB_G * B, TxtFoldArgs{}, 0,
                  SmallArgs{}, 1);
        SF_LAUNCH((pair_proj_score_kernel<2>), dim3(B), block, 0, st, ProjScoreArgs{}, FGlue{}, 0, va, sp, 0);
    }
    return launch_status();
}

extern "C" void sf_debug_trace(unsigned long long* buf) { g_trace = buf; }
extern "C" void sf_debug_force_write_through(int on) { g_force_sc1 = on; }

int pair_vis_small(const PanoSrc& src, int B, const float* vec, int ldvec, float* alpha, float* out,
                   int ldo, const Dropout& drop, int drop_col0, float* split_part,
                   unsigned* split_counter, const SmallPlan& b, hipStream_t st, int phase) {
    if (!pair_vis_small_accepts(b.inst(), phase)) return SF_ERR_UNSUPPORTED;
    if (!split_part || (phase == 0 && !split_counter) || !split_rows_fit(shape(src), B) || !aligned4(ldvec, ldo))
        return SF_ERR_UNSUPPORTED;
    if (half_misuse(src)) return SF_ERR_ARG;
    VisArgs va{src, vec, ldvec, alpha, out, ldo, drop, drop_col0};
    const int nv = (phase == 2 ? 1 : VSP_G) * B, nb = b.gx * b.gy;
    const dim3 grid(nv + nb), block(SMALL_WAVES * 64);
    const VisSplit sp{split_part, split_counter, g_trace};
    return launched(with_index<VIS_SMALL_INSTS>(vis_small_inst(b.inst(), phase), [&](auto i) {
        constexpr VisSmallInst I = VIS_SMALL_INST[decltype(i)::value];
        constexpr int M = I.mt, C = I.cpw, P = I.phase;
        if constexpr (P != 2) {
            if (src.half) {
                SF_LAUNCH_AS((inst_name<pair_vis_small_kernel<M, C, P, false, true>, M, C, P, false>(
                                 "pair_vis_small_kernel", P ? ", 1 != 2" : ", 0 != 2")),
                             (pair_vis_small_kernel<M, C, P, false, true>), grid, block, 0, st, va, sp, nv, b.args, b.gx);
                return;
            }
        }
        SF_LAUNCH_INST(pair_vis_small_kernel, (M, C, P), grid, block, 0, st, va, sp, nv, b.args, b.gx);
    }));
}

}
```

### speaker_follower_amd/csrc/sf_kernels.h

```cpp
#pragma once
#include "sf_common.h"
#include "sf_gemm.h"
#include "sf_lstm.h"
#include "sf_lstm_pw.h"
#include "sf_rows.h"
#include "sf_attention_plan.h"

namespace sf {

int visual_attn(int mode, const PanoSrc& src, int B, const float* vec, int ldvec, float* alpha,
                float* out, int ldo, const Dropout& drop, int drop_col0, hipStream_t st,
                float* split_part = nullptr, unsigned* split_counter = nullptr, const double* vec64 = nullptr,
                int vec_slabs = 0, long vec_slab_stride = 0);
bool visual_attn_f64_supported(const PanoSrc& src, int B);

int linear_f64(const float* A32, const double* A64, int lda, const float* W, int ldw, const float* bias, int M, int N,
               int K, double* y64, int ldy64, float* y32, int ldy32, hipStream_t st);
int linear_f64_w64(const float* A32, int lda, const double* W, int ldw, const double* bias, int M, int N, int K,
                   double* y64, int ldy64, float* y32, int ldy32, hipStream_t st);
extern int g_precise_attention;
int text_attn_fwd(const float* ctx, const uint8_t* mask, int B, int L, int H, const float* t,
                  int ldt, float* alpha, float* wc, int ldwc, hipStream_t st,
                  const int32_t* ctx_row = nullptr);
int text_attn_bwd(const float* ctx, int B, int L, int H, const float* dwc, int lddwc,
// ... 82 lines not shown
int sum_accum(const float* s, int M, float* out, hipStream_t st);
int fill(float* p, size_t n, float v, hipStream_t st);
int cotenant(int blocks, int threads, int lds_bytes, long long ticks, float* sink, hipStream_t st);
int flag_wait(const unsigned* flag, unsigned target, hipStream_t st);
int flag_set(unsigned* flag, unsigned value, hipStream_t st);
int adam_step(float* p, const float* g, float* m, float* v, size_t n, double lr, double beta1,
              double beta2, double eps, double wd, int step, hipStream_t st);
int adam_step_dev(float* p, const float* g, float* m, float* v, size_t n, double lr, double beta1, double beta2,
                  double eps, double wd, int* step_dev, float* coef, const unsigned* guard, hipStream_t st);
struct RowMoves {
    struct M { const float* src; float* dst; const int* idx; int lds, ldd, w, scatter; } m[4];
    int n;
};
int move_rows(const RowMoves& mv, int n, hipStream_t st);
struct FillRegions {
    struct R { void* ptr; unsigned long long count, value; int width; } r[8];
    int n;
};
int fill_regions(const FillRegions& fr, hipStream_t st);
int site_advance(uint32_t* word, uint32_t by, hipStream_t st);
int store_u32x4(uint32_t* dst, uint32_t a, uint32_t b, uint32_t c, uint32_t d, hipStream_t st);
int transpose(const float* src, int R, int C, float* dst, hipStream_t st);
int transpose_ld(const float* src, int lds, int R, int C, float* dst, hipStream_t st);
int dropout_tm(float* x, int T, int B, int E, const Dropout& d, const int* rev, hipStream_t st);
int embedding_bwd(const float* demb, int ldd, const int64_t* seq, int Lpad, int T, int B, int E, int padding_idx,
                  const Dropout& d, const int* rev, float* grad, hipStream_t st);
int embedding_tm(const float* table, int E, const int64_t* seq, int B, int Lpad, int T, float* out,
                 hipStream_t st);
int embedding_rows(const float* table, int E, const int64_t* idx, int B, float* out,
                   hipStream_t st);
int ctx_grad_slice(const float* dctx, int T, int H, int B, int t, const Dropout& d, float* out,
                   hipStream_t st);

int gather_panorama(const PanoSrc& s, int B, float* out, hipStream_t st);
int gather_candidates(const CandSrc& s, int B, float* all_u, float* is_valid, hipStream_t st);
int gather_actions(const CandSrc& s, int B, const int* a, float* out, hipStream_t st, int ldo = 0);
int gather_path_actions(const float* table, int V, int IMG, int LOC, const int* vp, const int* act_view,
                        const float* sincos, const int* act, int N, float* out, int ldo, hipStream_t st,
                        int half = 0);

int reverse_tokens(const int64_t* seq, int Lpad, const int* lengths, int B, int64_t* out, hipStream_t st);
int bi_assemble(const float* ctx_f, const float* ctx_r, const int* lengths, int B, int T, int H, const Dropout& d,
                float* out, hipStream_t st);
int bi_split(const float* dctx, const int* lengths, int B, int T, int H, const Dropout& d, float* dctx_f,
             float* dctx_r, hipStream_t st);
int gather_rows(const float* src, int lds, const int* idx, int n, int w, float* dst, int ldd,
                hipStream_t st);
int scatter_rows(const float* src, int lds, const int* idx, int n, int w, float* dst, int ldd,
                 hipStream_t st);
int logprob_topk(float* logit, int ld, int N, int n, const int* n_valid, int k, int* idx,
                 float* logp, hipStream_t st);
int speaker_beam_select(const sf_spk_beam& s, const int32_t* top_w, const float* top_lp, const float* alpha,
                        hipStream_t st);
int follower_beam_select(const sf_fol_beam& s, const int32_t* top_a, const float* top_lp, const float* alpha,
                         hipStream_t st);
int state_factored_select(const sf_state_search& s, const float* logp, int ld_logp, int32_t* dev_in, hipStream_t st);
bool state_factored_select_supported(const sf_state_search& s);

struct SmallPlan;
int pair_small_small(const SmallPlan& a, const SmallPlan& b, hipStream_t st);
int pair_small_text(const SmallPlan& a, const float* ctx, const uint8_t* mask, int B, int L, int H,
                    const float* t, int ldt, float* alpha, float* wc, int ldwc,
                    const int32_t* ctx_row, hipStream_t st);
int pair_visbwd_small(const PanoSrc& src, int B, const float* vec, int ldvec, float* alpha, float* out,
                      int ldo, const Dropout& drop, int drop_col0, const SmallPlan& b, hipStream_t st, int vec_slabs = 0,
                      long vec_slab_stride = 0);
int pair_vis_small(const PanoSrc& src, int B, const float* vec, int ldvec, float* alpha, float* out,
                   int ldo, const Dropout& drop, int drop_col0, float* split_part,
                   unsigned* split_counter, const SmallPlan& b, hipStream_t st, int phase = 0);

int pair_textfold_small_small(const float* ctx_q, const float* ctx_o, const uint8_t* mask, int B, int L, int H,
                              const float* vec, int ldvec, float* part, unsigned* counter, float* z, int ldz, float* alpha,
                              const SmallPlan& a, const SmallPlan& b, hipStream_t st);
int pair_apro_small(const SmallPlan& a, const SmallPlan& b, hipStream_t st);
struct FGlue;
int pair_score_merge(const CandSrc& src, int B, int D, const float* r, const float* wt, const float* b_a,
                     const float* b_out, const FGlue& g, const PanoSrc& psrc, float* alpha, float* out, int ldo,
                     const Dropout& drop, int drop_col0, float* split_part, hipStream_t st);

struct ProjTables {
    const float *pv, *pa, *lv, *la;
    int ld, H;
};
bool proj_chain_supported(const CandSrc& us, const PanoSrc* xn, int B, int H, int L, const ProjTables& pt);
int proj_attention_alone(const PanoSrc& x, int B, const ProjTables& pt, const float* h1, int ldh1, float* alpha, float* out,
                         int ldo, int late, float* split_part, unsigned* counter, hipStream_t st);
int visual_attn_proj(const CandSrc& us, const PanoSrc& x, int B, int H, int L, const ProjTables& pt, const float* h, int ldh,
                     float* alpha, float* out, int ldo, const Dropout& drop, int drop_col0, float* split_part,
                     unsigned* counter, hipStream_t st);
extern int g_proj_text_groups;
void proj_text_slots_warm();
int pair_proj_textfold(const float* ctx_q, const float* ctx_o, const uint8_t* mask, int B, int L, int H, const float* vec,
                       int ldvec, float* part, unsigned* counter, float* z, int ldz, float* alpha, const SmallPlan& y,
                       const CandSrc& us, const PanoSrc* xn, const ProjTables& pt, const float* h1, int ldh1, float* split_part,
                       hipStream_t st);
int pair_proj_score(const CandSrc& us, int B, int H, int L, const ProjTables& pt, const float* z, int ldz, const float* y, int ldy,
                    const FGlue& g, const PanoSrc* xn, int vphase, const float* h1, int ldh1, float* alpha, float* out, int ldo,
                    const Dropout& drop, int drop_col0, float* split_part, unsigned* counter, hipStream_t st);

struct FGlue;
int follower_glue_fwd(const FGlue& g, hipStream_t st);
int score_glue_fwd(const CandSrc& src, int B, int D, const float* r, const float* wt,
                   const float* b_a, const float* b_out, const FGlue& g, hipStream_t st);
int softmax_ce_bwd(int B, int N, int ld, const float* logit, const int64_t* target, int ignore,
                   const float* gscale, float* dlogit, hipStream_t st, int rps = 0);
int speaker_glue_fwd(int B, int vocab, int ldv, const float* logit, const int64_t* target,
                     int feedback, int pad_idx, int eos_idx, uint8_t* ended, int64_t* w_t,
                     float* score, float* nll_term, float* live, hipStream_t st, const sf_sample* sample = nullptr,
                     int rps = 0);
int speaker_sample_max_vocab();
int speaker_loss_finalize(const float* sum_cnt, const int64_t* words, int eos, int T, int B, float* loss, float* gscale,
                          hipStream_t st);
int reduce_terms(const float* term, const float* live, int T, int B, float* sum_cnt,
                 hipStream_t st);
int loss_finalize(const float* sum_cnt, int T, float* loss, float* gscale, hipStream_t st);

}
```

### speaker_follower_amd/features.py

```python
import base64
import csv
import ctypes as C
import json
import sys
import weakref

import numpy as np
import torch

from . import _lib
from ._lib import call
from .runtime import ptr, stream

NUM_VIEWS = 36
MEAN_POOLED_DIM = 2048
LOC_DIM = 128
ANGLE_INC = np.pi / 6.0


def build_loc_table(n_views=NUM_VIEWS, loc=LOC_DIM):
    g = loc // 4
    tab = np.zeros((n_views, n_views, loc), np.float32)
    for view in range(n_views):
        for abs_view in range(n_views):
            rel = (abs_view - view) % 12 + (abs_view // 12) * 12
            h = (rel % 12) * ANGLE_INC
            e = (rel // 12 - 1) * ANGLE_INC
            tab[view, abs_view, 0:g] = np.sin(h)
            tab[view, abs_view, g:2 * g] = np.cos(h)
            tab[view, abs_view, 2 * g:3 * g] = np.sin(e)
            tab[view, abs_view, 3 * g:] = np.cos(e)
    return tab


def cand_sincos(rel_heading, rel_elevation):
    h = np.asarray(rel_heading, np.float64)
    e = np.asarray(rel_elevation, np.float64)
    return np.stack((np.sin(h), np.cos(h), np.sin(e), np.cos(e)), axis=-1).astype(np.float32)


DTYPES = {'fp32': torch.float32, 'fp16': torch.float16}
FILE_DTYPES = {'fp32': 'float32', 'fp16': 'float16'}
CHECK_ROWS = 256


def _dtype_name(dtype):
    if dtype not in DTYPES:
        raise ValueError("dtype must be 'fp32' or 'fp16' (got %r)" % (dtype,))
    return dtype


def round_to_fp16(rows, row0=0):
    half = rows.to(torch.float16)
    bad = ~torch.isfinite(half.reshape(half.shape[0], -1)).all(dim=1)
    if bool(bad.any()):
        r = int(torch.nonzero(bad)[0, 0])
        raise ValueError('feature table row %d does not fit fp16 storage: it holds a NaN, an infinity or a magnitude '
                         'that rounds to infinity (fp16 max is 65504)' % (row0 + r))
    return half


def tsv_to_bin(tsv_path, bin_path, dtype='fp32'):
    half = _dtype_name(dtype) == 'fp16'
    csv.field_size_limit(sys.maxsize)
    names = ['scanId', 'viewpointId', 'image_w', 'image_h', 'vfov', 'features']
    ids = []
    with open(tsv_path, 'rt') as f, open(bin_path, 'wb') as out:
        for item in csv.DictReader(f, delimiter='\t', fieldnames=names):
            buf = base64.b64decode(item['features'])
            if len(buf) != NUM_VIEWS * MEAN_POOLED_DIM * 4:
                raise ValueError('row %s_%s: %d feature bytes' % (item['scanId'], item['viewpointId'], len(buf)))
            if half:
                row = torch.from_numpy(np.frombuffer(buf, np.float32).reshape(1, NUM_VIEWS, MEAN_POOLED_DIM).copy())
                buf = round_to_fp16(row, len(ids)).numpy().tobytes()
            out.write(buf)
            ids.append(item['scanId'] + '_' + item['viewpointId'])
    meta = {'ids': ids, 'shape': [len(ids), NUM_VIEWS, MEAN_POOLED_DIM]}
    if half:
        meta['dtype'] = FILE_DTYPES['fp16']
    with open(bin_path + '.json', 'w') as f:
        json.dump(meta, f)
    return len(ids)


def _forget_projected(addr, pv):
    if pv is not None:
        cur = _lib.Projected()
        if not _lib.lib.sf_projected_registered(C.c_void_p(addr), C.byref(cur)) or cur.pv != pv:
            return
    _lib.lib.sf_projected_register(C.c_void_p(addr), None)


class FeatureStore:

    def __init__(self, table, ids=None, device='cuda', loc=LOC_DIM, dtype='fp32'):
        self.dtype = _dtype_name(dtype)
        if isinstance(table, np.ndarray):
            if table.dtype != np.float16:
                table = np.ascontiguousarray(table, np.float32)
            table = torch.from_numpy(np.ascontiguousarray(table))
        if table.dim() != 3:
            raise ValueError('feature table must be [n, V, IMG] (got %s)' % (tuple(table.shape),))
        if self.dtype == 'fp16' and table.dtype != torch.float16:
            out = torch.empty(table.shape, dtype=torch.float16, device=device)
            for r0 in range(0, table.shape[0], CHECK_ROWS):
                out[r0:r0 + CHECK_ROWS].copy_(round_to_fp16(table[r0:r0 + CHECK_ROWS].to(torch.float32), r0))
            self.table = out
        else:
            self.table = table.to(device=device, dtype=DTYPES[self.dtype]).contiguous()
            if self.dtype == 'fp16':
                for r0 in range(0, self.table.shape[0], CHECK_ROWS):
                    round_to_fp16(self.table[r0:r0 + CHECK_ROWS], r0)
        self.n, self.V, self.IMG = self.table.shape
        if self.dtype == 'fp16' and self.IMG % 4:
            raise ValueError('fp16 storage needs IMG %% 4 == 0 (got %d)' % self.IMG)
        if self.table.numel():
            addr = self.table.data_ptr()
            call('sf_feature_table_f16', C.c_void_p(addr), 1 if self.dtype == 'fp16' else 0)
            if self.dtype == 'fp16':
                weakref.finalize(self, _lib.lib.sf_feature_table_f16, C.c_void_p(addr), 0)
            call('sf_projected_register', C.c_void_p(addr), None)
        self._projected = weakref.WeakKeyDictionary()
        self.LOC = loc
        self.F = self.IMG + loc
        self.device = self.table.device
        self.loc_table = torch.from_numpy(build_loc_table(self.V, loc)).to(self.device)
        self.index = {k: i for i, k in enumerate(ids)} if ids is not None else None

    @classmethod
    def from_tsv(cls, path, device='cuda', dtype='fp32'):
        csv.field_size_limit(sys.maxsize)
        names = ['scanId', 'viewpointId', 'image_w', 'image_h', 'vfov', 'features']
        ids, rows = [], []
        with open(path, 'rt') as f:
            for item in csv.DictReader(f, delimiter='\t', fieldnames=names):
                ids.append(item['scanId'] + '_' + item['viewpointId'])
                buf = base64.b64decode(item['features'])
                rows.append(np.frombuffer(buf, np.float32).reshape(NUM_VIEWS, MEAN_POOLED_DIM))
        return cls(np.stack(rows), ids, device, dtype=dtype)

    @classmethod
    def from_bin(cls, path, device='cuda', chunk_rows=512, dtype=None):
        with open(path + '.json') as f:
            meta = json.load(f)
        n, V, IMG = meta['shape']
        stored = meta.get('dtype', FILE_DTYPES['fp32'])
        if stored not in FILE_DTYPES.values():
            raise ValueError('%s.json: unknown dtype %r' % (path, stored))
        file16 = stored == FILE_DTYPES['fp16']
        dtype = _dtype_name(('fp16' if file16 else 'fp32') if dtype is None else dtype)
        mm = np.memmap(path, dtype=np.float16 if file16 else np.float32, mode='r', shape=(n, V, IMG))
        table = torch.empty(n, V, IMG, dtype=DTYPES[dtype], device=device)
        for r0 in range(0, n, chunk_rows):
            r1 = min(n, r0 + chunk_rows)
            rows = torch.from_numpy(np.array(mm[r0:r1]))
            if dtype == 'fp16':
                rows = round_to_fp16(rows, r0)
            table[r0:r1].copy_(rows)
        return cls(table, meta['ids'], device, dtype=dtype)

    def row(self, scan_id, viewpoint_id):
        return self.index[scan_id + '_' + viewpoint_id]

    def rows_f32(self, idx):
        return self.table[idx].to(torch.float32)

    def projected(self, decoder, build=True):
        from .model import decoder_fold, decoder_params
        from .runtime import weight_key, ws_args
        if self.dtype != 'fp32' or not self.table.numel() or self.IMG % 4 or self.LOC % 16:
            return None
        hit = self._projected.get(decoder)
        if hit is None and not build:
            return None
        params = decoder_params(decoder)
        key = weight_key(*(params[i] for i in (4, 5, 6, 10, 11, 12, 13, 14, 15))) + \
            (self.table.data_ptr(), self.table._version, self.loc_table.data_ptr())
        if hit is None or hit['key'] != key:
            H = decoder.hidden_size
            if H % 4 or decoder.feature_size != self.F:
                return None
            ld, rows = int(_lib.lib.sf_projected_ld(H)), self.n * self.V
            new = lambda r: torch.empty(r, ld, device=self.device, dtype=torch.float32)
            bufs = hit['bufs'] if hit is not None and hit['bufs'][0].shape == (rows, ld) else \
                (new(rows), new(rows), new(self.V * self.V), new(5))
            fold = decoder_fold(decoder)
            rc = _lib.lib.sf_projected_build(C.byref(fold), ptr(self.table), rows, ptr(self.loc_table), self.V, self.IMG,
                                             self.LOC, H, *(ptr(b) for b in bufs), *ws_args(self.device))
            if rc == _lib.SF_ERR_UNSUPPORTED and hit is None:
                return None
            _lib.check(rc, 'sf_projected_build')
            struct = _lib.Projected(*(b.data_ptr() for b in bufs), self.loc_table.data_ptr(), params[4].data_ptr(),
                                    params[10].data_ptr(), H, ld, self.V, self.IMG, self.LOC, 0)
            first = hit is None
            hit = dict(key=key, bufs=bufs, struct=struct, builds=(0 if first else hit['builds']) + 1)
            self._projected[decoder] = hit
            if first:
                addr = self.table.data_ptr()
                weakref.finalize(decoder, _forget_projected, addr, bufs[0].data_ptr())
                weakref.finalize(self, _forget_projected, addr, None)
        call('sf_projected_register', C.c_void_p(self.table.data_ptr()), C.byref(hit['struct']))
        return hit

    def note_unprojected(self, decoder):
        if decoder not in self._projected:
            self._projected[decoder] = None

    def seen_unprojected(self, decoder):
        return decoder in self._projected and self._projected[decoder] is None

    def pano(self, vp, view):
        return _lib.Pano(None, self.table.data_ptr(), self.loc_table.data_ptr(), vp.data_ptr(),
                         view.data_ptr(), self.V, self.IMG, self.LOC)

    def cands(self, vp, cand_view, sincos, a_num, A):
        return _lib.Cands(None, self.table.data_ptr(), vp.data_ptr(), cand_view.data_ptr(),
                          sincos.data_ptr(), a_num.data_ptr(), A, self.V, self.IMG, self.LOC)

    def gather_panorama(self, vp, view):
        B = vp.shape[0]
        out = torch.empty(B, self.V, self.F, device=self.device, dtype=torch.float32)
        p = self.pano(vp, view)
        call('sf_gather_panorama', C.byref(p), B, ptr(out), stream())
        return out

    def gather_candidates(self, vp, cand_view, sincos, a_num):
        B, A = cand_view.shape
        all_u = torch.empty(B, A, self.F, device=self.device, dtype=torch.float32)
        is_valid = torch.empty(B, A, device=self.device, dtype=torch.float32)
        c = self.cands(vp, cand_view, sincos, a_num, A)
        call('sf_gather_candidates', C.byref(c), B, ptr(all_u), ptr(is_valid), stream())
        return all_u, is_valid

    def gather_actions(self, vp, act_view, sincos, act):
        B = vp.shape[0]
        out = torch.empty(B, self.F, device=self.device, dtype=torch.float32)
        a_num = torch.full((B,), 2, dtype=torch.int32, device=self.device)
        cv = torch.stack((torch.zeros_like(act_view), act_view), 1).contiguous()
        sc = torch.stack((torch.zeros_like(sincos), sincos), 1).contiguous()
        c = self.cands(vp, cv, sc, a_num, 2)
        call('sf_gather_actions', C.byref(c), B, ptr(act), ptr(out), stream())
        return out
```

### speaker_follower_amd/follower.py

```python
import contextlib
import ctypes as C
from dataclasses import dataclass

import numpy as np
import torch

from . import _lib
from ._lib import call
from .features import cand_sincos
from .model import (decoder_params, decoder_w_struct, _encoder_structs, _TAPE_KEYS,
                    grad_ptr, trainable_embedding, bi_encoder_tapes, bi_encoder_fwd, bi_encoder_bwd)
from .runtime import ptr, stream, ws_args, wgrad_ws_args, ensure_workspace, dropout_arg, fill_regions, fault_bits, reissue_per_step, concurrent_stream, graph_capture, WeightsMoved, transposed, check_gate_weights, gate_weights_pass, register_bf16_weights
from .dp import collectives_on

byref = C.byref

PAD, UNK, EOS, BOS = 0, 1, 2, 3
FEEDBACK = {'teacher': 0, 'argmax': 1, 'sample': 2}


def batch_instructions_from_encoded(encoded_instructions, max_length, reverse=False, sort=False,
                                    device=None):
    first, src = {}, []
    for inst in encoded_instructions:
# ... 100 lines not shown
            if t < m:
                target[t, b] = acts[t]
    adj = [ob['adj_loc_list'] for ob in distinct]
    n_adj = np.array([len(x) for x in adj], np.int32)
    A = int(a_max or n_adj.max())
    D = len(distinct)
    d_vp, d_view = np.empty(D, np.int32), np.empty(D, np.int32)
    d_cv = np.zeros((D, A), np.int32)
    d_h, d_e = np.zeros((D, A), np.float64), np.zeros((D, A), np.float64)
    for k, (ob, cands) in enumerate(zip(distinct, adj)):
        d_vp[k], d_view[k] = ob['vp_row'], ob['viewIndex']
        for a, d in enumerate(cands[1:], 1):
            d_cv[k, a], d_h[k, a], d_e[k, a] = d['absViewIndex'], d['rel_heading'], d['rel_elevation']
    a_num = n_adj[at]
    bad = (target != -1) & ((target < 0) | (target >= a_num))
    if bad.any():
        t, b = np.argwhere(bad)[0]
        raise ValueError('route %d, step %d: action %d of %d candidates' % (b, t, target[t, b], a_num[t, b]))
    fb = FollowerBatch(instr=list(encoded_instructions), vp=d_vp[at], view=d_view[at], a_num=a_num,
                       cand_view=d_cv[at], cand_heading=d_h[at], cand_elevation=d_e[at], target=target, a_max=A)
    return fb, S


def scored_route_outputs(path_obs, path_actions, actions, step_scores, live):
    acts = np.asarray(actions).astype(np.int64)
    sc = np.asarray(step_scores, np.float32) * np.asarray(live, np.float32)
    S = acts.shape[0]
    ss = np.add.accumulate(sc, axis=0, dtype=np.float32)
    is0 = acts == 0
    last = np.where(is0.any(0), is0.argmax(0), S - 1).tolist()
    acts_l, sc_l, ss_l = acts.T.tolist(), sc.T.tolist(), ss.T.tolist()
    out = []
    for b, (obs, pa) in enumerate(zip(path_obs, path_actions)):
        k, m = last[b] + 1, len(pa)
        o0 = obs[0]
        steps = [o0] + [obs[t] for t in range(min(k, m))] + [obs[m - 1]] * max(0, k - m)
        out.append({'instr_id': o0['instr_id'],
                    'trajectory': [(ob['viewpoint'], ob['heading'], ob['elevation']) for ob in steps],
                    'actions': acts_l[b][:k], 'scores': sc_l[b][:k], 'observations': [o0],
                    'instr_encoding': o0['instr_encoding'], 'score': ss_l[b][k - 1]})
    return out


class RolloutState:
    pass


class _RolloutLossFn(torch.autograd.Function):

    @staticmethod
    def forward(ctx, engine, state, *params):
        ctx.engine, ctx.state = engine, state
        return state.loss_buf.clone().reshape(())

    @staticmethod
    def backward(ctx, dloss):
        if ctx.state is None:
            raise RuntimeError('second backward through a pass whose tape the first backward released')
        ctx.engine._backward(ctx.state, dloss)
        ctx.state = None
        return (None, None) + (None,) * (len(ctx.needs_input_grad) - 2)


PROJECT_MAX_B = 256


class projected_pass:

    def __init__(self, on):
        self.on = int(bool(on))

    def __enter__(self):
        self.prev = int(_lib.lib.sf_projected_is_used())
        if self.prev != self.on:
            _lib.lib.sf_projected_use(self.on)
        return self

    def __exit__(self, *exc):
        if self.prev != self.on:
            _lib.lib.sf_projected_use(self.prev)
        return False


class FollowerEngine:
    def __init__(self, encoder, decoder, store, group=None):
        self.encoder, self.decoder, self.store = encoder, decoder, store
        self.group = group
        self.iteration = 0
        self.site_next = 0
        self.site_word = None
        self.dropout_seed = None
        self.two_stream_backward = True
        self._side_stream = None
        self.grad_sync = None
        self._open_forks = []
        self.fold_text = True
        self.pipelined = True
        self.two_stream_forward = False
        self.episode_call = True
        self.fused_env_step = True
        self.fallbacks = 0
        self._gate_weights = 'fp32'
        self._project = 'auto'
        self._capturing = False

    @property
    def project(self):
        return self._project

    @project.setter
    def project(self, mode):
        if not (mode is True or mode is False or mode == 'auto'):
            raise ValueError("project must be 'auto', True or False, not %r" % (mode,))
        self._project = mode

    def _projected_tables(self, B, build=None, T=1, A=1):
        store = self.store
        if self._project is False or B > PROJECT_MAX_B or store.dtype != 'fp32':
            return None
        if not _lib.lib.sf_projected_supported(B, self.decoder.hidden_size, T, A, store.V, store.IMG, store.LOC):
            return None
        if build is None:
            build = self._project is True or (self._capturing and not self.store.seen_unprojected(self.decoder))
        hit = self.store.projected(self.decoder, build=build)
        if hit is None and self._project == 'auto' and not self._capturing:
            self.store.note_unprojected(self.decoder)
        return hit

    @property
    def gate_weights(self):
        return self._gate_weights

    @gate_weights.setter
    def gate_weights(self, mode):
        self._gate_weights = check_gate_weights(mode)

    def pass_gate_weights(self, train=None):
        if self._gate_weights == 'fp32':
            return 'fp32'
        enc, dec = self.encoder, self.decoder
        taped = (dec.training if train is None else train) or (torch.is_grad_enabled() and any(
            p.requires_grad for p in list(enc.parameters()) + list(dec.parameters())))
        return 'fp32' if taped else self._gate_weights

    def rollout(self, batch, steps, feedback='argmax', train=None, finalize=True):
        lstm = self.decoder.lstm
        with gate_weights_pass(self.pass_gate_weights(train), lstm.weight_ih, lstm.weight_hh):
            return self._rollout(batch, steps, feedback, train, finalize)

    def _rollout(self, batch, steps, feedback, train, finalize):
        enc, dec, store = self.encoder, self.decoder, self.store
        dev = store.device
        B, A, S = batch.batch_size, batch.a_max, steps
        bidir = enc.num_directions == 2
        H, E = enc.hidden_size * enc.num_directions, enc.embedding_size
        F, V = store.F, store.V
        D = dec.visual_attention_layer.linear_in_h.weight.shape[0]
        T = batch.mask.shape[1]
        Lpad = batch.seq.shape[1]
        training = dec.training if train is None else train
        new = lambda *s: torch.empty(*s, device=dev, dtype=torch.float32)
        st = RolloutState()
        st.batch, st.steps, st.dims = batch, S, (B, A, H, E, F, V, D, T)
        st.feedback = FEEDBACK[feedback]

        p_dec = dec.drop.p if training else 0.0
        p_enc = enc.drop.p if training else 0.0
        if self.dropout_seed is None:
            self.dropout_seed = torch.initial_seed() & 0xFFFFFFFF
        st.drop_dec = (p_dec, self.dropout_seed, batch.row0)
        st.drop_enc = (p_enc, self.dropout_seed ^ 0x5BD1E995, batch.row0)
        st.site0 = self.site_next
        st.site_stride = max(64, S + 2)
        self.site_next += st.site_stride
        self.iteration += 1
        st.site_dev = C.c_void_p(self.site_word.data_ptr()) if self.site_word is not None else None
        st.site_rel = 0 if self.site_word is not None else st.site0
        st.drop_dec += (st.site_dev, 1)
        st.drop_enc += (st.site_dev, 1)

        st.ctx = new(B, T, H)
        st.hs_all = new(steps + 1, B, H)
        st.cs_all = new(steps + 1, B, H)
        st.h_init, st.c_init = st.hs_all[0], st.cs_all[0]
        keep = training or (torch.is_grad_enabled() and any(
            p.requires_grad for p in list(enc.parameters()) + list(dec.parameters())))
        st.enc_tape = bi_encoder_tapes(B, T, E, H // 2, dev, keep) if bidir else \
            dict(emb=new(T, B, E) if keep else None, xg=new(T, B, 4 * H) if keep else None,
                 gates=new(T, B, 4 * H) if keep else None, hs=new(T + 1, B, H), cs=new(T + 1, B, H))
        etp = None if bidir else _lib.EncoderTape(*(st.enc_tape[k].data_ptr() if st.enc_tape[k] is not None else None
                                 for k in ('emb', 'xg', 'gates', 'hs', 'cs')))
        st.enc_table = not (keep and trainable_embedding(enc))
        if bidir:
            p_e, seed_e, row0 = st.drop_enc[:3]
            st.drop_enc_bi = (p_e, (seed_e + 0x9E3779B1 * row0) & 0xFFFFFFFF, 0, st.site_dev, 1)
            bi_encoder_fwd(enc, batch.seq, batch.lengths_dev, T, dropout_arg(*st.drop_enc_bi), st.site_rel,
                           st.enc_table, st.enc_tape, st.ctx, st.h_init, st.c_init)
        else:
            ew = _encoder_structs(enc, table=st.enc_table)
            call('sf_encoder_lstm_fwd', byref(ew), B, Lpad, T, E, H, ptr(batch.seq),
                 ptr(batch.lengths_dev), ptr(st.ctx), ptr(st.h_init), ptr(st.c_init), byref(etp),
                 dropout_arg(*st.drop_enc), st.site_rel, *ws_args(dev))

        shapes = dict(t_v=(D,), q=(F,), alpha_v=(V,), xin=(2 * F,), gates=(4 * H,), c1=(H,),
                      h1=(H,), cat2=(2 * H,), t_text=(H,), alpha=(T,), h_tilde=(H,), t_a=(D,),
                      wt=(D,), r=(F,), logit=(A,))
        shapes_x = dict(shapes, xin=(2 * F,))
        st.tape = {k: new(S + (1 if k == 'xin' else 0), B, *shapes_x[k]) for k in _TAPE_KEYS
                   if k not in ('h1', 'c1')}
        st.hs, st.cs = st.hs_all, st.cs_all
        st.tape['h1'], st.tape['c1'] = st.hs[1:], st.cs[1:]
        st.ended = torch.empty(B, dtype=torch.uint8, device=dev)
        fill_regions((st.tape['xin'][0], 0.0), (st.ended, 0))
        st.actions = torch.empty(S, B, dtype=torch.int64, device=dev)
        st.target_used = torch.empty(S, B, dtype=torch.int64, device=dev)
        st.step_scores, st.ce_term, st.live = new(S, B), new(S, B), new(S, B)
        st.sum_cnt, st.gscale, st.loss_buf = new(S, 2), new(S), new(1)
        params = decoder_params(dec)
        all_params = list(params) + [p for p in enc.parameters()]
        st.differentiable = torch.is_grad_enabled() and any(p.requires_grad for p in all_params)
        dw = decoder_w_struct(params)
        ws = ws_args(dev)
        d_dec = _lib.Dropout(float(st.drop_dec[0]), int(st.drop_dec[1]) & 0xFFFFFFFF, int(st.drop_dec[2]), st.site_dev, 1)
        d_ptr = C.pointer(d_dec) if st.drop_dec[0] else None
        on_device_env = hasattr(batch, 'advance')
        if on_device_env:
            batch.advance(-1)
        pipelined = self.pipelined and not on_device_env
        st.episode = None
        st.projected, st.projected_tables = False, None
        nav_episode = (on_device_env and self.pipelined and self.episode_call and self.fused_env_step
                       and bool(dw.visual.w_v_t))
        if (pipelined or nav_episode) and self.episode_call:
            ep = _lib.FollowerEpisode()
            ep.S, ep.B, ep.H, ep.D, ep.L, ep.A = S, B, H, D, T, A
            ep.X = store.pano(batch.vp[0], batch.view[0])
            ep.U = store.cands(batch.vp[0], batch.cand_view[0], batch.sincos[0], batch.a_num[0], A)
            ep.h_init, ep.c_init = st.h_init.data_ptr(), st.c_init.data_ptr()
            ep.ctx, ep.ctx_mask = st.ctx.data_ptr(), batch.mask.data_ptr()
            ep.tape = _lib.DecoderTape(*(st.tape[k][0].data_ptr() for k in _TAPE_KEYS))
            ep.glue = _lib.FollowerGlue(
                None, batch.target[0].data_ptr(), st.feedback, st.ended.data_ptr(),
                st.actions[0].data_ptr(), st.target_used[0].data_ptr(), st.step_scores[0].data_ptr(),
                None, 0, None, 0, st.ce_term[0].data_ptr(), st.live[0].data_ptr(),
                int(st.drop_dec[1]) ^ 0x1B873593, 0, batch.row0, st.site_dev)
            ep.drop = d_dec
            ep.step0 = st.site_rel
            ep.side_stream = None
            if nav_episode:
                st.navio0 = batch.fused_step(0)
                ep.glue.nav = C.cast(C.pointer(st.navio0), C.c_void_p)
            if self.two_stream_forward and not nav_episode:
                if self._side_stream is None:
                    self._side_stream = concurrent_stream(dev)
                ep.side_stream = self._side_stream.cuda_stream
            st.text_folded = (self.fold_text and not st.differentiable and not training
                              and ep.side_stream is None and S > 1 and T <= 80)
            if st.text_folded:
                st.ctx_fold = new(2, B, T, H)
                ep.ctx_q, ep.ctx_o = st.ctx_fold[0].data_ptr(), st.ctx_fold[1].data_ptr()
            st.projected_tables = self._projected_tables(B, T=T, A=A) if (st.text_folded and not nav_episode) else None
            with projected_pass(st.projected_tables is not None):
                before = _lib.lib.sf_projected_steps()
                call('sf_follower_episode_fwd', byref(dw), byref(ep), *ws)
                st.projected = _lib.lib.sf_projected_steps() > before
            st.episode = (ep, dw)
        tapes = [] if st.episode else [_lib.DecoderTape(*(st.tape[k][t].data_ptr() for k in _TAPE_KEYS))
                                       for t in range(S)]
        panos = [] if st.episode else [store.pano(batch.vp[t], batch.view[t]) for t in range(S)]
        if pipelined and not st.episode:
            call('sf_attn_decoder_head_fwd', byref(dw), byref(panos[0]), B, H, D, ptr(st.h_init),
                 byref(tapes[0]), d_ptr, st.site_rel, *ws)
        deferred = on_device_env and self.pipelined and dw.visual.w_v_t and not st.episode
        if deferred:
            call('sf_attn_decoder_head_fwd', byref(dw), byref(panos[0]), B, H, D, ptr(st.h_init),
                 byref(tapes[0]), d_ptr, st.site_rel, *ws)
        for t in range(0 if not st.episode else S, S):
            pano = panos[t]
            cnd = store.cands(batch.vp[t], batch.cand_view[t], batch.sincos[t], batch.a_num[t], A)
            tp = tapes[t]
            h0 = st.h_init if t == 0 else st.tape['h1'][t - 1]
            c0 = st.c_init if t == 0 else st.tape['c1'][t - 1]
            glue = _lib.FollowerGlue(
                None, batch.target[t].data_ptr(), st.feedback, st.ended.data_ptr(),
                st.actions[t].data_ptr(), st.target_used[t].data_ptr(), st.step_scores[t].data_ptr(),
                st.tape['xin'][t + 1].data_ptr(), 2 * F, d_ptr, 2 * (st.site_rel + t + 1),
                st.ce_term[t].data_ptr(), st.live[t].data_ptr(),
                int(st.drop_dec[1]) ^ 0x1B873593, st.site_rel + t, batch.row0, st.site_dev)
            navio = None
            if deferred and self.fused_env_step:
                navio = batch.fused_step(t)
                glue.nav = C.cast(C.pointer(navio), C.c_void_p)
            if pipelined or deferred:
                nxt = t + 1 < S
                call('sf_attn_decoder_tail_fwd', byref(dw), byref(cnd), B, H, D, T, None, ptr(h0),
                     ptr(c0), ptr(st.ctx), ptr(batch.mask), None, byref(tp), byref(glue), d_ptr,
                     st.site_rel + t, byref(panos[t + 1]) if nxt and not deferred else None,
                     byref(tapes[t + 1]) if nxt else None, *ws)
            else:
                call('sf_attn_decoder_fwd', byref(dw), byref(pano), byref(cnd), B, H, D, T, None,
                     ptr(h0), ptr(c0), ptr(st.ctx), ptr(batch.mask), None, byref(tp), byref(glue),
                     d_ptr, st.site_rel + t, *ws)
            if on_device_env:
                if navio is None:
                    batch.advance(t, st.actions[t], st.ended)
                if deferred and t + 1 < S:
                    call('sf_attn_decoder_attend_fwd', byref(panos[t + 1]), B, byref(tapes[t + 1]), d_ptr,
                         st.site_rel + t + 1, *ws)
        call('sf_reduce_terms', ptr(st.ce_term), ptr(st.live), S, B, ptr(st.sum_cnt), ws[2])
        st.logits = st.tape['logit']
        st.h, st.c = st.tape['h1'][S - 1], st.tape['c1'][S - 1]
        st.all_params = all_params
        if not finalize:
            return st
        if self.group is not None:
            table, grp = st.sum_cnt, self.group
            self._collective(lambda: torch.distributed.all_reduce(table, group=grp))
        return self.finish(st)

    collective_hook = None

    def _collective(self, action):
        if self.collective_hook is not None:
            self.collective_hook(action)
        else:
            action()

    def run(self, batch, steps, feedback='argmax', train=None, backward=False, while_running=None):
        dev = self.store.device
        site, it = self.site_next, self.iteration
        group = self.group if self.group is not None and collectives_on(self.group) else None

        def issue():
            st = self.rollout(batch, steps, feedback, train)
            if backward:
                st.loss.backward()
            return st

        st = issue()
        if while_running is not None:
            while_running()
        bits = fault_bits(dev, group)
        if bits:
            if backward:
                if self.grad_sync is not None:
                    self.grad_sync.abort()
                for p_ in st.all_params:
                    if p_.grad is not None:
                        p_.grad.zero_()
            self.site_next, self.iteration = site, it
            st = reissue_per_step(self.encoder, self, dev, 'a rollout', issue, bits, group)
        return st

    def finish(self, st, total=None):
        if total is not None:
            st.sum_cnt = total
        call('sf_loss_finalize', ptr(st.sum_cnt), st.steps, ptr(st.loss_buf), ptr(st.gscale), stream())
        if st.differentiable:
            st.loss = _RolloutLossFn.apply(self, st, *st.all_params)
        else:
            st.loss = st.loss_buf.reshape(())
        return st

    def _baked_pointers(self, gate_weights='fp32', projected=False):
        enc = self.encoder
        if enc.num_directions == 2:
            e2d = enc.encoder2decoder
            ew = b''.join(bytes(_encoder_structs(enc, direction=d)) for d in (0, 1)) + \
                repr((e2d.weight.data_ptr(), e2d.bias.data_ptr(), transposed(e2d.weight).data_ptr())).encode()
        else:
            ew = bytes(_encoder_structs(enc))
        dw = decoder_w_struct(decoder_params(self.decoder))
        packed = b''
        if gate_weights == 'bf16':
            lstm = self.decoder.lstm
            packed = repr(tuple(t.data_ptr() for t in register_bf16_weights(lstm.weight_ih, lstm.weight_hh))).encode()
        tables = b''
        if projected:
            hit = self.store.projected(self.decoder, build=False)
            tables = b'projected' + (bytes(hit['struct']) if hit is not None else b'')
        return ew + bytes(dw) + packed + tables

    @contextlib.contextmanager
    def _capture_policy(self):
        prev, self._capturing = self._capturing, True
        try:
            yield
        finally:
            self._capturing = prev

    def _guarded(self, graph_replay, projected=False):
        mode = self._gate_weights
        baked = self._baked_pointers(mode, projected)

        def replay():
            if self._baked_pointers(mode, projected) != baked:
                raise WeightsMoved('a weight (or one of its cached layouts) moved since this rollout was '
                                   'captured; capture() again')
            graph_replay()
        return replay

    def capture(self, batch, steps, feedback='argmax'):
        sampled = feedback == 'sample'
        ctl = torch.zeros(4, dtype=torch.int32, device=self.store.device) if sampled else None
        with torch.no_grad(), self._capture_policy():
            self.rollout(batch, steps, feedback, train=False)
            torch.cuda.synchronize()
            graph = torch.cuda.CUDAGraph()
            side = torch.cuda.Stream()
            ensure_workspace(side, self.store.device)
            side.wait_stream(torch.cuda.current_stream())
            keep = (self.site_next, self.iteration)
            self.site_word = ctl[0:1] if sampled else None
            try:
                with torch.cuda.stream(side):
                    with graph_capture(graph, side):
                        st = self.rollout(batch, steps, feedback, train=False)
            finally:
                self.site_word = None
            if sampled:
                self.site_next, self.iteration = keep
            torch.cuda.current_stream().wait_stream(side)
        st.capture_stream = side

        def graph_replay():
            if sampled:
                call('sf_store_u32x4', C.c_void_p(ctl.data_ptr()), int(self.site_next) & 0xFFFFFFFF, 0, 0, 0, stream())
                st.site0 = self.site_next
                self.site_next += st.site_stride
                self.iteration += 1
            graph.replay()
        return self._guarded(graph_replay, st.projected), st

    def capture_training(self, batch, steps, feedback='sample', optimizers=(), zero=None):
        from .runtime import TrainingGraph
        opts = list(optimizers)
        if self.group is not None or self.grad_sync is not None:
            if self.encoder.num_directions == 2:
                raise NotImplementedError('capture_training: a data-parallel iteration with a bidirectional encoder '
                                          'runs eagerly')
            return self._capture_training_dp(batch, steps, feedback, opts, zero)

        def body():
            if zero is not None:
                zero.zero()
            else:
                for o in opts:
                    o.zero_grad()
            st = self.rollout(batch, steps, feedback, train=True)
            st.loss.backward()
            for o in opts:
                o.step()
            return st
        return TrainingGraph(self, body, opts, self.store.device)

    def _capture_training_dp(self, batch, steps, feedback, opts, zero):
        from .runtime import TrainingGraph
        sync = self.grad_sync
        if sync is None:
            raise ValueError('a data-parallel capture needs engine.grad_sync (dp.BucketedGrads: the buffer the '
                             'all-reduces work on)')
        zero = zero if zero is not None else sync
        dev = self.store.device

        def body():
            zero.zero()
            with torch.no_grad():
                st = self.rollout(batch, steps, feedback, train=True)
                self._backward(st, torch.ones((), device=dev))
            sync.wait()
            for o in opts:
                o.step()
            return st
        return TrainingGraph(self, body, opts, dev, segmented=(sync,))

    def capture_sharded(self, shards, steps, feedback='argmax'):
        dev = self.store.device
        streams = [torch.cuda.Stream() for _ in shards]
        graphs, states = [], []
        with torch.no_grad(), self._capture_policy():
            for sh, s in zip(shards, streams):
                s.wait_stream(torch.cuda.current_stream())
                with torch.cuda.stream(s):
                    self.rollout(sh, steps, feedback, train=False)
                    torch.cuda.synchronize()
                    g = torch.cuda.CUDAGraph()
                    with graph_capture(g, s):
                        states.append(self.rollout(sh, steps, feedback, train=False, finalize=False))
                graphs.append(g)
            torch.cuda.synchronize()
        total = torch.empty(steps, 2, device=dev)
        loss_buf = torch.empty(1, device=dev)
        gscale = torch.empty(steps, device=dev)

        def replay_all():
            cur = torch.cuda.current_stream()
            for s, g in zip(streams, graphs):
                s.wait_stream(cur)
                with torch.cuda.stream(s):
                    g.replay()
            for s in streams:
                cur.wait_stream(s)
            total.copy_(states[0].sum_cnt)
            for st in states[1:]:
                call('sf_add_f32', ptr(total), ptr(st.sum_cnt), total.numel(), stream())
            call('sf_loss_finalize', ptr(total), steps, ptr(loss_buf), ptr(gscale), stream())

        return self._guarded(replay_all, any(st.projected for st in states)), states, loss_buf

    def _backward(self, st, dloss):
        enc, dec, store = self.encoder, self.decoder, self.store
        batch, S = st.batch, st.steps
        B, A, H, E, F, V, D, T = st.dims
        dev = store.device
        new = lambda *s: torch.empty(*s, device=dev, dtype=torch.float32)
        gscale = st.gscale * dloss.to(torch.float32)
        params = decoder_params(dec)
        dw, dg = decoder_w_struct(params), decoder_w_struct(params, grad=True)
        gshapes = dict(dgates=(4 * H,), dpre=(H,), dt_text=(H,), dt_v=(D,), dq=(F,), dwt=(D,),
                       dta=(D,), dr=(F,), dc=())
        gkeys = ('dgates', 'dpre', 'dt_text', 'dt_v', 'dq', 'dwt', 'dta', 'dr', 'dc')
        gt = {k: new(S, B, *gshapes[k]) for k in gkeys}
        dlogit = new(B, A)
        dh_a, dc_a, dh_b, dc_b = new(B, H), new(B, H), new(B, H), new(B, H)
        dctx = torch.zeros(B, T, H, device=dev, dtype=torch.float32)
        ws = ws_args(dev)
        d_dec = _lib.Dropout(float(st.drop_dec[0]), int(st.drop_dec[1]) & 0xFFFFFFFF, int(st.drop_dec[2]), st.site_dev, 1)
        d_ptr = C.pointer(d_dec) if st.drop_dec[0] else None
        dh1 = dc1 = None
        if st.episode is not None:
            ep, _ = st.episode
            gt_dcat2, gt_ds, gt_dh1d = new(S, B, 2 * H), new(S, B, T), new(S, B, H)
            gt0e = _lib.DecoderGTape(*(gt[k].data_ptr() for k in gkeys), gt_dcat2.data_ptr(), gt_ds.data_ptr(),
                                     gt_dh1d.data_ptr())
            if self.two_stream_backward and (self._side_stream is not None or not torch.cuda.is_current_stream_capturing()):
                if self._side_stream is None:
                    self._side_stream = concurrent_stream(dev)
                ep.side_stream = self._side_stream.cuda_stream
            else:
                ep.side_stream = None
            which = C.c_int(0)
            call('sf_follower_episode_bwd', byref(dw), byref(ep), byref(gt0e), ptr(gscale), ptr(dlogit),
                 ptr(dh_a), ptr(dc_a), ptr(dh_b), ptr(dc_b), ptr(dctx), byref(which), *ws)
            dh1, dc1 = (dh_b, dc_b) if which.value else (dh_a, dc_a)
        for t in range(S - 1 if st.episode is None else -1, -1, -1):
            pano = store.pano(batch.vp[t], batch.view[t])
            cnd = store.cands(batch.vp[t], batch.cand_view[t], batch.sincos[t], batch.a_num[t], A)
            tp = _lib.DecoderTape(*(st.tape[k][t].data_ptr() for k in _TAPE_KEYS))
            gtp = _lib.DecoderGTape(*(gt[k][t].data_ptr() for k in gkeys), None, None, None)
            call('sf_follower_glue_bwd', B, A, ptr(st.tape['logit'][t]), ptr(st.target_used[t]),
                 ptr(gscale[t:t + 1]), ptr(dlogit), ws[2])
            call('sf_attn_decoder_bwd', byref(dw), None, byref(pano), byref(cnd), B, H, D, T,
                 ptr(st.hs[t]), ptr(st.cs[t]), ptr(st.ctx), byref(tp), byref(gtp), ptr(dlogit),
                 ptr(dh1), ptr(dc1), ptr(dh_a), ptr(dc_a), ptr(dctx), d_ptr, st.site_rel + t, *ws)
            dh1, dc1 = dh_a, dc_a
            dh_a, dc_a, dh_b, dc_b = dh_b, dc_b, dh_a, dc_a
        sync = self.grad_sync
        tp0 = _lib.DecoderTape(*(st.tape[k].data_ptr() for k in _TAPE_KEYS))
        gt0 = _lib.DecoderGTape(*(gt[k].data_ptr() for k in gkeys), None, None, None)
        overlap = self.two_stream_backward and (self._side_stream is not None or not torch.cuda.is_current_stream_capturing())
        if overlap:
            side = self._side_stream
            if side is None:
                side = self._side_stream = concurrent_stream(dev)
            side.wait_stream(torch.cuda.current_stream())
            self._open_forks = [side]
        try:
            if overlap:
                self._issue_wgrad(side, dw, dg, params, S * B, H, D, F, st, tp0, gt0, dev, sync)
            else:
                self._decoder_wgrad(dw, dg, params, S * B, H, D, F, st, tp0, gt0, wgrad_ws_args(dev), sync)
            if enc.num_directions == 2:
                bi_encoder_bwd(enc, batch.seq, batch.lengths_dev, T, dropout_arg(*st.drop_enc_bi), st.site_rel,
                               st.enc_table, st.enc_tape, st.h_init, dctx, dh1, dc1)
            else:
                etp = _lib.EncoderTape(*(st.enc_tape[k].data_ptr() for k in ('emb', 'xg', 'gates', 'hs', 'cs')))
                ew = _encoder_structs(enc, table=st.enc_table)
                eg = _encoder_structs(enc, grad=True, seq=None if st.enc_table else batch.seq)
                call('sf_encoder_lstm_bwd', byref(ew), byref(eg), B, T, E, H, ptr(batch.lengths_dev),
                     ptr(st.h_init), ptr(dctx), ptr(dh1), ptr(dc1), byref(etp), dropout_arg(*st.drop_enc),
                     st.site_rel, *ws)
            if sync is not None:
                sync.launch(2)
            if overlap:
                torch.cuda.current_stream().wait_stream(side)
        finally:
            self._open_forks = []

    def _issue_wgrad(self, side, dw, dg, params, M, H, D, F, st, tp0, gt0, dev, sync):
        with torch.cuda.stream(side):
            self._decoder_wgrad(dw, dg, params, M, H, D, F, st, tp0, gt0, wgrad_ws_args(dev), sync)
# ... 14 lines not shown
```

Before: 1.432 million agent-steps/s.

## Precompute per-viewpoint LSTM input-gate rows and gather them in the score kernel

Builds a table holding W_ih·image_features for every (viewpoint, view) row, plus a small table of location-encoding gate contributions. The score kernel that picks the next action now gathers the chosen row, combines it with the sin/cos terms, and writes the next step's input-gate preactivation. The next LSTM step then only multiplies the remaining input columns and h, skipping the large 2048-wide image GEMM each decode step. The cost is a large precomputed table (n_rows × 4H floats) that must be rebuilt whenever the weights change, extra registration and guard logic, and falling off the fused LSTM-step path.

```diff
diff --git a/include/sf_hip.h b/include/sf_hip.h
--- a/include/sf_hip.h
+++ b/include/sf_hip.h
@@ -503,6 +503,18 @@
 long long sf_projected_steps(void);
 int sf_projected_supported(int B, int H, int L, int A, int V, int IMG, int LOC);
 void sf_debug_projected_chunk_rows(int rows);
+typedef struct sf_gate_rows {
+    const float *gu, *gl;
+    const float* key_w;
+    int32_t H, V, IMG, LOC;
+} sf_gate_rows;
+int sf_gate_rows_build(const float* w_ih, const float* table, long long n_rows, int IMG, int LOC, int H, float* gu, float* gl,
+                       void* ws, size_t ws_bytes, sf_stream stream);
+int sf_gate_rows_register(const void* table, const sf_gate_rows* g);
+int sf_gate_rows_registered(const void* table, sf_gate_rows* out);
+void sf_gate_rows_use(int on);
+int sf_gate_rows_is_used(void);
+long long sf_gate_rows_steps(void);
 void sf_debug_projected_partials_late(int on);
 int sf_projected_text_groups_plan(int B, int L, int with_partials, int slots, int product_blocks, int* grid);
 void sf_debug_projected_text_groups(int groups);
diff --git a/speaker_follower_amd/csrc/sf_api.hip b/speaker_follower_amd/csrc/sf_api.hip
--- a/speaker_follower_amd/csrc/sf_api.hip
+++ b/speaker_follower_amd/csrc/sf_api.hip
@@ -106,6 +106,24 @@
 }
 inline int projected_ld(int H) { return (H + 1 + 3) & ~3; }
 
+constexpr int GATE_TABLES = 16;
+struct GateEntry { const void* table; sf_gate_rows g; };
+GateEntry g_gate[GATE_TABLES];
+int g_gate_n = 0;
+std::mutex g_gate_mutex;
+std::atomic<int> g_gate_use{1};
+std::atomic<long long> g_gate_steps{0};
+bool gate_rows_lookup(const void* table, sf_gate_rows* out) {
+    if (!table || !g_gate_use.load(std::memory_order_relaxed)) return false;
+    std::lock_guard<std::mutex> lock(g_gate_mutex);
+    for (int i = 0; i < g_gate_n; ++i)
+        if (g_gate[i].table == table) {
+            *out = g_gate[i].g;
+            return true;
+        }
+    return false;
+}
+
 inline PanoSrc pano(const sf_pano* p) {
     return PanoSrc{p->dense, p->table, p->loc_table, p->vp, p->view, p->V, p->IMG, p->LOC,
                    p->dense ? 0 : table_is_f16(p->table)};
@@ -199,23 +217,25 @@
 
 int lstm_fwd_i(const sf_lstm_w* w, int B, int I, int H, const float* x, int ldx, const float* h0,
                const float* c0, float* h1, float* c1, float* gates, float* h1_drop, int ld_h1_drop,
-               const Dropout& drop, Arena ar, hipStream_t st) {
+               const Dropout& drop, Arena ar, hipStream_t st,
+               const float* xg = nullptr, int x_col0 = 0) {
     LstmPwFwd p{};
-    p.xg = nullptr; p.b_ih = w->b_ih; p.b_hh = w->b_hh;
+    p.xg = xg; p.b_ih = w->b_ih; p.b_hh = w->b_hh;
     p.c0 = c0; p.h0 = h0; p.B = B; p.H = H; p.gates = gates; p.h1 = h1; p.c1 = c1;
     p.h1_drop = h1_drop; p.ld_h1_drop = ld_h1_drop; p.drop = drop; p.lengths = nullptr;
-    if (I + H <= 1024 && H % 16 == 0) {
+    if (!xg && I + H <= 1024 && H % 16 == 0) {
         LstmStepArgs f{};
         f.h0 = h0; f.w_hh = w->w_hh; f.x = x; f.ldx = ldx; f.w_ih = w->w_ih; f.I = I; f.xg = nullptr;
         f.b_ih = w->b_ih; f.b_hh = w->b_hh; f.B = B; f.H = H; f.pw = p;
         return lstm_step_fused(f, st);
     }
-    Seg segs[2] = {{x, ldx, w->w_ih, I, I}, {h0, H, w->w_hh, H, H}};
+    if (!xg) x_col0 = 0;
+    Seg segs[2] = {{x + x_col0, ldx, w->w_ih + x_col0, I, I - x_col0}, {h0, H, w->w_hh, H, H}};
     LinearOut o{};
     float* slabs = nullptr;
     int ks = 1;
     const void* packed[2];
-    const bool bf16w = bf16_packed(w->w_ih, w->w_hh, packed);
+    const bool bf16w = !xg && bf16_packed(w->w_ih, w->w_hh, packed);
     TRY(linear_nt(segs, 2, B, 4 * H, o, ar.rest(), ar.rest_n(), st, &slabs, &ks, bf16w ? packed : nullptr));
     p.slabs = slabs; p.ks = ks;
     return lstm_pointwise_fwd(p, st);
@@ -610,6 +630,55 @@
     TRY(linear_plain(loc_table, LOC, wt_v + IMG, F, nullptr, V * V, ld, LOC, EPI_NONE, lv, ld, ar, st));
     return linear_plain(sel, Ks, wt_a + IMG, Fa, nullptr, 5, ld, Ks, EPI_NONE, la, ld, ar, st);
 }
+int sf_gate_rows_build(const float* w_ih, const float* table, long long n_rows, int IMG, int LOC, int H, float* gu, float* gl,
+                       void* ws, size_t ws_bytes, sf_stream stream) {
+    SF_ENTER();
+    SF_CHECK_ARG(w_ih && table && gu && gl && n_rows > 0 && IMG > 0 && IMG % 4 == 0 && LOC > 0 && LOC % 16 == 0 && H > 0 &&
+                 H % 4 == 0);
+    if (table_is_f16(table)) return SF_ERR_UNSUPPORTED;
+    const int F = IMG + LOC, G = 4 * H, g = LOC / 4;
+    Arena ar = arena(ws, ws_bytes);
+    hipStream_t st = S(stream);
+    float* sel = ar.take((size_t)4 * LOC);
+    NEED(sel);
+    TRY(fill(sel, (size_t)4 * LOC, 0.f, st));
+    for (int q = 0; q < 4; ++q) TRY(fill(sel + (size_t)q * LOC + (size_t)q * g, (size_t)g, 1.f, st));
+    for (long long r0 = 0; r0 < n_rows; r0 += g_proj_chunk_rows) {
+        const int m = (int)std::min<long long>(g_proj_chunk_rows, n_rows - r0);
+        TRY(linear_plain(table + (size_t)r0 * IMG, IMG, w_ih, 2 * F, nullptr, m, G, IMG, EPI_NONE, gu + (size_t)r0 * G, G, ar, st));
+    }
+    return linear_plain(sel, LOC, w_ih + IMG, 2 * F, nullptr, 4, G, LOC, EPI_NONE, gl, G, ar, st);
+}
+int sf_gate_rows_register(const void* table, const sf_gate_rows* g) {
+    SF_CHECK_ARG(table);
+    if (g) SF_CHECK_ARG(g->gu && g->gl && g->key_w && g->H > 0 && g->H % 4 == 0 && g->V > 0 && g->IMG > 0 && g->LOC > 0);
+    std::lock_guard<std::mutex> lock(g_gate_mutex);
+    int at = -1;
+    for (int i = 0; i < g_gate_n; ++i)
+        if (g_gate[i].table == table) at = i;
+    if (!g) {
+        if (at >= 0) g_gate[at] = g_gate[--g_gate_n];
+        return SF_OK;
+    }
+    if (at < 0) {
+        if (g_gate_n == GATE_TABLES) return SF_ERR_UNSUPPORTED;
+        at = g_gate_n++;
+    }
+    g_gate[at] = GateEntry{table, *g};
+    return SF_OK;
+}
+int sf_gate_rows_registered(const void* table, sf_gate_rows* out) {
+    std::lock_guard<std::mutex> lock(g_gate_mutex);
+    for (int i = 0; i < g_gate_n; ++i)
+        if (table && g_gate[i].table == table) {
+            if (out) *out = g_gate[i].g;
+            return 1;
+        }
+    return 0;
+}
+void sf_gate_rows_use(int on) { g_gate_use.store(on ? 1 : 0, std::memory_order_relaxed); }
+int sf_gate_rows_is_used(void) { return g_gate_use.load(std::memory_order_relaxed); }
+long long sf_gate_rows_steps(void) { return g_gate_steps.load(std::memory_order_relaxed); }
 void sf_gate_product_bf16_weights(int on) { g_bf16w_on.store(on ? 1 : 0, std::memory_order_relaxed); }
 int sf_gate_product_bf16_weights_is_on(void) { return g_bf16w_on.load(std::memory_order_relaxed); }
 int sf_gate_product_bf16_supported(int M, int K1, int K2, int N) {
@@ -844,6 +913,13 @@
     const int32_t* ctx_row;
     Arena ar;
     hipStream_t st;
+    struct GateStep* gate;
+};
+
+struct GateStep {
+    const float* xg_in;
+    GateRows rows;
+    bool wrote;
 };
 
 static inline int issued(int rc) { return rc == SF_ERR_UNSUPPORTED ? SF_ERR_LAUNCH : rc; }
@@ -925,9 +1001,13 @@
     TRY(pair_proj_textfold(tf.ctx_q, tf.ctx_o, s.ctx_mask, B, s.L, H, tp->cat2 + H, 2 * H, f.tpart, f.tcount, f.zbuf, f.ldp,
                            tp->alpha, py, s.us, s.paired && !late ? &s.xn : nullptr, pt, tp->h1, H, f.part, s.st));
     g_proj_steps.fetch_add(1, std::memory_order_relaxed);
-    return issued(pair_proj_score(s.us, B, H, s.L, pt, f.zbuf, f.ldp, f.ybuf, f.ldp, make_glue(s.us, B, tp->logit, s.glue),
-                                  s.paired ? &s.xn : nullptr, late ? 0 : 2, tp->h1, H, s.paired ? tn->alpha_v : nullptr,
-                                  s.paired ? tn->xin + F : nullptr, 2 * F, s.dn_in, F, f.part, af.tickets(), s.st));
+    const bool gate = s.gate && s.gate->rows.xg_next && s.paired;
+    TRY(issued(pair_proj_score(s.us, B, H, s.L, pt, f.zbuf, f.ldp, f.ybuf, f.ldp, make_glue(s.us, B, tp->logit, s.glue),
+                               s.paired ? &s.xn : nullptr, late ? 0 : 2, tp->h1, H, s.paired ? tn->alpha_v : nullptr,
+                               s.paired ? tn->xin + F : nullptr, 2 * F, s.dn_in, F, f.part, af.tickets(), s.st,
+                               gate ? &s.gate->rows : nullptr)));
+    if (gate) s.gate->wrote = true;
+    return SF_OK;
 }
 
 static int tail_fold4(const TailStep& s, const TextFold& tf) {
@@ -1055,10 +1135,11 @@
                           const uint8_t* ctx_mask, const int32_t* ctx_row, const sf_decoder_tape* tp,
                           const sf_follower_glue* glue, const sf_dropout* drop, uint32_t step_id,
                           const sf_pano* X_next, const sf_decoder_tape* tn, void* ws, size_t ws_bytes,
-                          sf_stream stream, const TextFold* tf = nullptr) {
+                          sf_stream stream, const TextFold* tf = nullptr, GateStep* gate = nullptr) {
     SF_CHECK_ARG(w && U && h0 && c0 && ctx && tp && B > 0 && L > 0 && (!glue || glue_ok(U, glue)) &&
                  (!X_next || tn));
     TailStep s{};
+    s.gate = gate;
     s.w = w; s.us = cands(U); s.B = B; s.H = H; s.D = D; s.L = L; s.F = s.us.IMG + s.us.LOC;
     s.tp = tp; s.tn = tn; s.glue = glue;
     s.ctx = ctx; s.ctx_mask = ctx_mask; s.ctx_row = ctx_row;
@@ -1073,8 +1154,10 @@
     s.last_step = !X_next && !tn;
     const Dropout d_in = make_dropout(drop, 2 * step_id, 2);
     if (u_prev) TRY(dropout_copy(u_prev, s.F, B, s.F, tp->xin, 2 * s.F, d_in, 0, s.st));
+    const float* xg = gate && !u_prev ? gate->xg_in : nullptr;
     TRY(lstm_fwd_i(&w->lstm, B, 2 * s.F, H, tp->xin, 2 * s.F, h0, c0, tp->h1, tp->c1, tp->gates,
-                   tp->cat2 + H, 2 * H, s.d_h, s.ar, s.st));
+                   tp->cat2 + H, 2 * H, s.d_h, s.ar, s.st, xg, s.F));
+    if (xg) g_gate_steps.fetch_add(1, std::memory_order_relaxed);
     return tail_dispatch(s, tf);
 }
 
@@ -1438,15 +1521,39 @@
         }
         return fk.join();
     }
+    float* xg_buf[2] = {nullptr, nullptr};
+    sf_gate_rows gr{};
+    {
+        const CandSrc us0 = cands(&cur.U);
+        const PanoSrc x0 = pano(&cur.X);
+        const int F = us0.IMG + us0.LOC;
+        const size_t row = ((size_t)e->B * 4 * e->H + 63) & ~(size_t)63;
+        const Arena whole = arena(ws, ws_bytes);
+        ProjTables pt;
+        const void* packed[2];
+        if (tf && !nav0 && !drop && e->S > 1 && e->B <= VIS_SPLIT_MAX_B && !us0.dense && !us0.half &&
+            gate_rows_lookup(us0.table, &gr) && gr.key_w == w->lstm.w_ih && gr.H == e->H && gr.V == us0.V &&
+            gr.IMG == us0.IMG && gr.LOC == us0.LOC && e->H % 4 == 0 && F % 4 == 0 && 2 * F + e->H > 1024 &&
+            projected_for(w, us0, &x0, e->B, e->H, e->L, &pt) && !bf16_packed(w->lstm.w_ih, w->lstm.w_hh, packed) &&
+            whole.tk && 2 * row <= whole.cap / 8) {
+            xg_buf[0] = (float*)ws;
+            xg_buf[1] = xg_buf[0] + row;
+            ws = xg_buf[1] + row;
+            ws_bytes -= 2 * row * sizeof(float);
+        }
+    }
+    const float* xg_in = nullptr;
     for (int t = 0; t < e->S; ++t) {
         const bool more = t + 1 < e->S;
         StepView nxt = more ? step_view(e, t + 1) : cur;
         const sf_nav_io nv = nav0 ? nav_view(nav0, e, t) : sf_nav_io{};
         if (nav0) cur.glue.nav = &nv;
         const StepState in = state_in(e, t);
+        GateStep gs{xg_in, GateRows{gr.gu, gr.gl, more ? xg_buf[t & 1] : nullptr}, false};
         TRY(decoder_tail_i(w, &cur.U, e->B, e->H, e->D, e->L, nullptr, in.h, in.c, e->ctx, e->ctx_mask,
                            nullptr, &cur.tp, &cur.glue, drop, e->step0 + t, more && !nav0 ? &nxt.X : nullptr,
-                           more ? &nxt.tp : nullptr, ws, ws_bytes, stream, tf));
+                           more ? &nxt.tp : nullptr, ws, ws_bytes, stream, tf, xg_buf[0] ? &gs : nullptr));
+        xg_in = gs.wrote ? gs.rows.xg_next : nullptr;
         if (nav0 && more)
             TRY(sf_attn_decoder_attend_fwd(&nxt.X, e->B, &nxt.tp, drop, e->step0 + t + 1, ws, ws_bytes, stream));
         cur = nxt;
diff --git a/speaker_follower_amd/csrc/sf_attention.hip b/speaker_follower_amd/csrc/sf_attention.hip
--- a/speaker_follower_amd/csrc/sf_attention.hip
+++ b/speaker_follower_amd/csrc/sf_attention.hip
@@ -929,6 +929,9 @@
     const float* z;
     const float* y;
     int ldz, ldy;
+    const float* gu;
+    const float* gl;
+    float* xg_next;
 };
 
 __device__ __forceinline__ void proj_score_glue_body(const ProjScoreArgs& a, const FGlue& g, int b) {
@@ -988,25 +991,40 @@
         if (lane == 0 && ac < A) s_logit[ac] = d + cst;
     }
     __syncthreads();
+    const bool gate = a.xg_next != nullptr;
+    const int gc = gate ? min(tid, H - 1) : 0, gs = gate ? H : 0;
+    const float4* glp = reinterpret_cast<const float4*>(gate ? a.gl : a.la);
+    const float4 gl0 = glp[gc], gl1 = glp[gs + gc], gl2 = glp[2 * gs + gc], gl3 = glp[3 * gs + gc];
     if (wave == 0) {
         const int at = follower_glue_row(g, b, lane < A ? s_logit[lane] : 0.f, gin);
         if (lane == 0) s_at = at;
         if (g.nav.on && lane < A) nav_advance_slot(g.nav, b, lane, at, gin.was_ended || at == 0);
     }
     __syncthreads();
+    const int at = min(max(s_at, 0), A - 1);
+    const bool zero = at == 0 || at >= an || vp < 0;
+    const int view = __shfl(cvl, at, WAVE);
+    const float c0 = __shfl(scl.x, at, WAVE), c1 = __shfl(scl.y, at, WAVE), c2 = __shfl(scl.z, at, WAVE),
+                c3 = __shfl(scl.w, at, WAVE);
+    const size_t trow = (size_t)max(vp, 0) * V + min(max(view, 0), V - 1);
+    float4 gw = (gate ? reinterpret_cast<const float4*>(a.gu) + trow * H : glp)[gc];
     if (g.u_next) {
-        const int at = min(max(s_at, 0), A - 1);
         const int n4 = (a.src.IMG + a.src.LOC) >> 2;
         CandRow row;
-        row.zero = at == 0 || at >= an || vp < 0;
+        row.zero = zero;
         row.I4 = a.src.IMG >> 2;
         row.g4 = max(a.src.LOC >> 4, 1);
-        const int view = __shfl(cvl, at, WAVE);
-        row.img = reinterpret_cast<const float4*>(a.src.table) + ((size_t)max(vp, 0) * V + min(max(view, 0), V - 1)) * row.I4;
+        row.img = reinterpret_cast<const float4*>(a.src.table) + trow * row.I4;
         row.img16 = nullptr;
-        row.s0 = __shfl(scl.x, at, WAVE); row.s1 = __shfl(scl.y, at, WAVE);
-        row.s2 = __shfl(scl.z, at, WAVE); row.s3 = __shfl(scl.w, at, WAVE);
+        row.s0 = c0; row.s1 = c1; row.s2 = c2; row.s3 = c3;
         for (int c = tid; c < n4; c += NW * 64) store_u_next(g, b, c, cand_load<false>(row, c, !row.zero, n4));
+    }
+    if (gate && tid < H) {
+        f4fma(gw, c0, gl0);
+        f4fma(gw, c1, gl1);
+        f4fma(gw, c2, gl2);
+        f4fma(gw, c3, gl3);
+        reinterpret_cast<float4*>(a.xg_next)[(size_t)b * H + tid] = zero ? f4zero() : gw;
     }
 }
 
@@ -1513,10 +1531,13 @@
 
 int pair_proj_score(const CandSrc& us, int B, int H, int L, const ProjTables& pt, const float* z, int ldz, const float* y, int ldy,
                     const FGlue& g, const PanoSrc* xn, int vphase, const float* h1, int ldh1, float* alpha, float* out, int ldo,
-                    const Dropout& drop, int drop_col0, float* split_part, unsigned* counter, hipStream_t st) {
+                    const Dropout& drop, int drop_col0, float* split_part, unsigned* counter, hipStream_t st,
+                    const GateRows* gate) {
     if (!proj_chain_supported(us, xn, B, H, L, pt) || !aligned4(ldz, ldy, ldh1)) return SF_ERR_UNSUPPORTED;
     if (xn && (!split_part || !aligned4(ldo) || (vphase != 0 && vphase != 2) || (vphase == 0 && !counter))) return SF_ERR_UNSUPPORTED;
-    const ProjScoreArgs a{us, pt.pa, pt.la, pt.ld, H, z, y, ldz, ldy};
+    if (gate && (!gate->gu || !gate->gl || !gate->xg_next)) return SF_ERR_UNSUPPORTED;
+    ProjScoreArgs a{us, pt.pa, pt.la, pt.ld, H, z, y, ldz, ldy};
+    if (gate) { a.gu = gate->gu; a.gl = gate->gl; a.xg_next = gate->xg_next; }
     const VisArgs va = xn ? proj_vis_args(*xn, pt, h1, ldh1, alpha, out, ldo, drop, drop_col0) : VisArgs{};
     const VisSplit sp{split_part, counter, g_trace};
     const dim3 block(SMALL_WAVES * 64);
diff --git a/speaker_follower_amd/csrc/sf_kernels.h b/speaker_follower_amd/csrc/sf_kernels.h
--- a/speaker_follower_amd/csrc/sf_kernels.h
+++ b/speaker_follower_amd/csrc/sf_kernels.h
@@ -188,6 +188,10 @@
     const float *pv, *pa, *lv, *la;
     int ld, H;
 };
+struct GateRows {
+    const float *gu, *gl;
+    float* xg_next;
+};
 bool proj_chain_supported(const CandSrc& us, const PanoSrc* xn, int B, int H, int L, const ProjTables& pt);
 int proj_attention_alone(const PanoSrc& x, int B, const ProjTables& pt, const float* h1, int ldh1, float* alpha, float* out,
                          int ldo, int late, float* split_part, unsigned* counter, hipStream_t st);
@@ -202,7 +206,8 @@
                        hipStream_t st);
 int pair_proj_score(const CandSrc& us, int B, int H, int L, const ProjTables& pt, const float* z, int ldz, const float* y, int ldy,
                     const FGlue& g, const PanoSrc* xn, int vphase, const float* h1, int ldh1, float* alpha, float* out, int ldo,
-                    const Dropout& drop, int drop_col0, float* split_part, unsigned* counter, hipStream_t st);
+                    const Dropout& drop, int drop_col0, float* split_part, unsigned* counter, hipStream_t st,
+                    const GateRows* gate = nullptr);
 
 struct FGlue;
 int follower_glue_fwd(const FGlue& g, hipStream_t st);
diff --git a/speaker_follower_amd/features.py b/speaker_follower_amd/features.py
--- a/speaker_follower_amd/features.py
+++ b/speaker_follower_amd/features.py
@@ -37,6 +37,12 @@
     h = np.asarray(rel_heading, np.float64)
     e = np.asarray(rel_elevation, np.float64)
     return np.stack((np.sin(h), np.cos(h), np.sin(e), np.cos(e)), axis=-1).astype(np.float32)
+
+
+def gate_loc_groups(w_loc):
+    w = np.asarray(w_loc, np.float64)
+    g = w.shape[1] // 4
+    return np.stack([w[:, k * g:(k + 1) * g].sum(axis=1) for k in range(4)])
 
 
 DTYPES = {'fp32': torch.float32, 'fp16': torch.float16}
@@ -89,6 +95,14 @@
         if not _lib.lib.sf_projected_registered(C.c_void_p(addr), C.byref(cur)) or cur.pv != pv:
             return
     _lib.lib.sf_projected_register(C.c_void_p(addr), None)
+
+
+def _forget_gate_rows(addr, gu):
+    if gu is not None:
+        cur = _lib.GateRows()
+        if not _lib.lib.sf_gate_rows_registered(C.c_void_p(addr), C.byref(cur)) or cur.gu != gu:
+            return
+    _lib.lib.sf_gate_rows_register(C.c_void_p(addr), None)
 
 
 class FeatureStore:
@@ -120,7 +134,9 @@
             if self.dtype == 'fp16':
                 weakref.finalize(self, _lib.lib.sf_feature_table_f16, C.c_void_p(addr), 0)
             call('sf_projected_register', C.c_void_p(addr), None)
+            call('sf_gate_rows_register', C.c_void_p(addr), None)
         self._projected = weakref.WeakKeyDictionary()
+        self._gate_rows = weakref.WeakKeyDictionary()
         self.LOC = loc
         self.F = self.IMG + loc
         self.device = self.table.device
@@ -202,6 +218,36 @@
         call('sf_projected_register', C.c_void_p(self.table.data_ptr()), C.byref(hit['struct']))
         return hit
 
+    def gate_rows(self, decoder, build=True):
+        from .model import decoder_params
+        from .runtime import weight_key, ws_args
+        if self.dtype != 'fp32' or not self.table.numel() or self.IMG % 4 or self.LOC % 16:
+            return None
+        hit = self._gate_rows.get(decoder)
+        if hit is None and not build:
+            return None
+        w_ih = decoder_params(decoder)[0]
+        key = weight_key(w_ih) + (self.table.data_ptr(), self.table._version)
+        if hit is None or hit['key'] != key:
+            H = decoder.hidden_size
+            if H % 4 or decoder.feature_size != self.F or tuple(w_ih.shape) != (4 * H, 2 * self.F):
+                return None
+            rows = self.n * self.V
+            new = lambda r: torch.empty(r, 4 * H, device=self.device, dtype=torch.float32)
+            bufs = hit['bufs'] if hit is not None and hit['bufs'][0].shape == (rows, 4 * H) else (new(rows), new(4))
+            call('sf_gate_rows_build', ptr(w_ih), ptr(self.table), rows, self.IMG, self.LOC, H, ptr(bufs[0]), ptr(bufs[1]),
+                 *ws_args(self.device))
+            struct = _lib.GateRows(bufs[0].data_ptr(), bufs[1].data_ptr(), w_ih.data_ptr(), H, self.V, self.IMG, self.LOC)
+            first = hit is None
+            hit = dict(key=key, bufs=bufs, struct=struct, builds=(0 if first else hit['builds']) + 1)
+            self._gate_rows[decoder] = hit
+            if first:
+                addr = self.table.data_ptr()
+                weakref.finalize(decoder, _forget_gate_rows, addr, bufs[0].data_ptr())
+                weakref.finalize(self, _forget_gate_rows, addr, None)
+        call('sf_gate_rows_register', C.c_void_p(self.table.data_ptr()), C.byref(hit['struct']))
+        return hit
+
     def note_unprojected(self, decoder):
         if decoder not in self._projected:
             self._projected[decoder] = None
diff --git a/speaker_follower_amd/follower.py b/speaker_follower_amd/follower.py
--- a/speaker_follower_amd/follower.py
+++ b/speaker_follower_amd/follower.py
@@ -206,6 +206,23 @@
         return False
 
 
+class gate_rows_pass:
+
+    def __init__(self, on):
+        self.on = int(bool(on))
+
+    def __enter__(self):
+        self.prev = int(_lib.lib.sf_gate_rows_is_used())
+        if self.prev != self.on:
+            _lib.lib.sf_gate_rows_use(self.on)
+        return self
+
+    def __exit__(self, *exc):
+        if self.prev != self.on:
+            _lib.lib.sf_gate_rows_use(self.prev)
+        return False
+
+
 class FollowerEngine:
     def __init__(self, encoder, decoder, store, group=None):
         self.encoder, self.decoder, self.store = encoder, decoder, store
@@ -226,6 +243,7 @@
         self.fallbacks = 0
         self._gate_weights = 'fp32'
         self._project = 'auto'
+        self.gate_rows = True
         self._capturing = False
 
     @property
@@ -250,6 +268,11 @@
         if hit is None and self._project == 'auto' and not self._capturing:
             self.store.note_unprojected(self.decoder)
         return hit
+
+    def _gate_rows_tables(self, projected, train):
+        if projected is None or not self.gate_rows or self.pass_gate_weights(train) != 'fp32':
+            return None
+        return self.store.gate_rows(self.decoder, build=self._project is True or self._capturing)
 
     @property
     def gate_weights(self):
@@ -353,6 +376,7 @@
         pipelined = self.pipelined and not on_device_env
         st.episode = None
         st.projected, st.projected_tables = False, None
+        st.gate_rows, st.gate_rows_tables = False, None
         nav_episode = (on_device_env and self.pipelined and self.episode_call and self.fused_env_step
                        and bool(dw.visual.w_v_t))
         if (pipelined or nav_episode) and self.episode_call:
@@ -384,10 +408,12 @@
                 st.ctx_fold = new(2, B, T, H)
                 ep.ctx_q, ep.ctx_o = st.ctx_fold[0].data_ptr(), st.ctx_fold[1].data_ptr()
             st.projected_tables = self._projected_tables(B, T=T, A=A) if (st.text_folded and not nav_episode) else None
-            with projected_pass(st.projected_tables is not None):
-                before = _lib.lib.sf_projected_steps()
+            st.gate_rows_tables = self._gate_rows_tables(st.projected_tables, training)
+            with projected_pass(st.projected_tables is not None), gate_rows_pass(st.gate_rows_tables is not None):
+                before, gate_before = _lib.lib.sf_projected_steps(), _lib.lib.sf_gate_rows_steps()
                 call('sf_follower_episode_fwd', byref(dw), byref(ep), *ws)
                 st.projected = _lib.lib.sf_projected_steps() > before
+                st.gate_rows = _lib.lib.sf_gate_rows_steps() > gate_before
             st.episode = (ep, dw)
         tapes = [] if st.episode else [_lib.DecoderTape(*(st.tape[k][t].data_ptr() for k in _TAPE_KEYS))
                                        for t in range(S)]
@@ -486,7 +512,7 @@
             st.loss = st.loss_buf.reshape(())
         return st
 
-    def _baked_pointers(self, gate_weights='fp32', projected=False):
+    def _baked_pointers(self, gate_weights='fp32', projected=False, gate_rows=False):
         enc = self.encoder
         if enc.num_directions == 2:
             e2d = enc.encoder2decoder
@@ -503,6 +529,9 @@
         if projected:
             hit = self.store.projected(self.decoder, build=False)
             tables = b'projected' + (bytes(hit['struct']) if hit is not None else b'')
+        if gate_rows:
+            hit = self.store.gate_rows(self.decoder, build=False)
+            tables += b'gate_rows' + (bytes(hit['struct']) if hit is not None else b'')
         return ew + bytes(dw) + packed + tables
 
     @contextlib.contextmanager
@@ -513,12 +542,12 @@
         finally:
             self._capturing = prev
 
-    def _guarded(self, graph_replay, projected=False):
+    def _guarded(self, graph_replay, projected=False, gate_rows=False):
         mode = self._gate_weights
-        baked = self._baked_pointers(mode, projected)
+        baked = self._baked_pointers(mode, projected, gate_rows)
 
         def replay():
-            if self._baked_pointers(mode, projected) != baked:
+            if self._baked_pointers(mode, projected, gate_rows) != baked:
                 raise WeightsMoved('a weight (or one of its cached layouts) moved since this rollout was '
                                    'captured; capture() again')
             graph_replay()
@@ -554,7 +583,7 @@
                 self.site_next += st.site_stride
                 self.iteration += 1
             graph.replay()
-        return self._guarded(graph_replay, st.projected), st
+        return self._guarded(graph_replay, st.projected, st.gate_rows), st
 
     def capture_training(self, batch, steps, feedback='sample', optimizers=(), zero=None):
         from .runtime import TrainingGraph
@@ -630,7 +659,7 @@
                 call('sf_add_f32', ptr(total), ptr(st.sum_cnt), total.numel(), stream())
             call('sf_loss_finalize', ptr(total), steps, ptr(loss_buf), ptr(gscale), stream())
 
-        return self._guarded(replay_all, any(st.projected for st in states)), states, loss_buf
+        return self._guarded(replay_all, any(st.projected for st in states), any(st.gate_rows for st in states)), states, loss_buf
 
     def _backward(self, st, dloss):
         enc, dec, store = self.encoder, self.decoder, self.store
```

After: 1.507 million agent-steps/s (median of 6 runs). 1.05x the previous value.
